# pananananas/MVD

Hardware: AMD Instinct MI355X
Metric: UNet forward-passes/sec @512x512 SD2.1+MV adapter (higher is better)
Workload: dtype bf16; 1 GPU; cfg4: configs[3]/[4]: 8 objects x 4 target views per GPU (32 pairs), camera FiLM + cross-view adapter; pairs_per_gpu=32, global_pairs=32, latent=64x64x4, image=512x512, forward=cold, hip_graph=False, q2_statistics=replica-local, parallelism=dp1 (pairs sharded by object), weights=synthetic seeded, SD2.1 shapes (865.9M UNet x2 + 99.2M adapter + 19.1M camera), encoder_weights=distinct

## Files before the change

### include/mvd_hip.h

```cpp
#ifndef MVD_HIP_H
#define MVD_HIP_H
#include <stddef.h>
#include <stdint.h>

#ifdef __cplusplus
extern "C" {
#endif

#define MVD_MAX_LEVELS 4

typedef struct {
  int in_channels;
  int out_channels;
  int num_levels;
  int block_out_channels[MVD_MAX_LEVELS];
  int num_heads[MVD_MAX_LEVELS];
  int layers_per_block;
  int cross_attention_dim;
  int norm_num_groups;
  float norm_eps;
  int cam_output_dim;
  int cam_hidden_dim;
  int simple_cam_encoder;
  float cam_modulation_strength;
} mvd_config_t;

typedef struct mvd_engine mvd_engine_t;

const char* mvd_last_error(void);

int mvd_engine_create(const mvd_config_t* cfg, mvd_engine_t** out);
int mvd_engine_destroy(mvd_engine_t* e);

int mvd_engine_set_weight(mvd_engine_t* e, int set, const char* slot, const void* ptr, int64_t numel, int dtype);
int mvd_engine_clear_weights(mvd_engine_t* e, int set);

int64_t mvd_engine_workspace_bytes(mvd_engine_t* e, int batch, int height, int width, int text_len, int ref_batch);
int64_t mvd_engine_refcache_bytes(mvd_engine_t* e, int ref_batch, int height, int width, int keep_features);
int mvd_engine_bind_workspace(mvd_engine_t* e, void* ws, int64_t ws_bytes, void* refcache, int64_t refcache_bytes);

enum {
  MVD_USE_CAMERA = 1,
  MVD_USE_IMAGE = 2,
  MVD_REUSE_REF = 4,
  MVD_KEEP_FEATURES = 8,
  MVD_SHARE_REF = 16
};


typedef struct {
  int batch;
  int height, width;
  int text_len;
  const float* sample;
  const float* timesteps;
  const float* text;
  const float* source_camera;
  const float* target_camera;
  int cam_rows;
  int cam_batch;
  const float* fourier_proj;
  const float* source_latents;
  const float* encoder_text;
  int ref_batch;
  int flags;
  float* out;
  int views;
} mvd_forward_args_t;

int mvd_unet_forward(mvd_engine_t* e, const mvd_forward_args_t* args, void* stream);
int64_t mvd_engine_workspace_bytes_args(mvd_engine_t* e, const mvd_forward_args_t* args);

int mvd_unet_forward_objects(mvd_engine_t* e, const mvd_forward_args_t* args, int objects, void* stream);
int64_t mvd_engine_workspace_bytes_objects(mvd_engine_t* e, const mvd_forward_args_t* args, int objects);

int mvd_unet_forward_ragged(mvd_engine_t* e, const mvd_forward_args_t* args, const int* view_counts, int objects, void* stream);
int64_t mvd_engine_workspace_bytes_ragged(mvd_engine_t* e, const mvd_forward_args_t* args, const int* view_counts, int objects);

int64_t mvd_engine_reference_pixels(mvd_engine_t* e, int height, int width);
int mvd_engine_reference_encode(mvd_engine_t* e, const mvd_forward_args_t* args, float* local_stats, void* stream);
int mvd_engine_reference_finish(mvd_engine_t* e, const float* mean_k, void* stream);

int mvd_engine_set_graph(mvd_engine_t* e, int enable);

int mvd_engine_share_encoder_weights(mvd_engine_t* e, int enable);

int mvd_engine_set_freeu(mvd_engine_t* e, float s1, float s2, float b1, float b2);
int mvd_engine_clear_freeu(mvd_engine_t* e);

int mvd_engine_set_profiling(mvd_engine_t* e, int enable);
int mvd_engine_profile_summary(mvd_engine_t* e, int cap, int* cls, int* launches, double* ms, double* flops, double* bytes);
int mvd_engine_profile_shapes(mvd_engine_t* e, char* buf_host, int cap);

int mvd_engine_num_features(mvd_engine_t* e);
int mvd_engine_feature_shape(mvd_engine_t* e, int idx, int* channels, int* height, int* width);
int mvd_engine_get_feature(mvd_engine_t* e, int idx, float* out_nchw, void* stream);
int mvd_engine_encode_cameras(mvd_engine_t* e, const float* source_camera, const float* target_camera, int cam_rows,
                              int batch, const float* fourier_proj, float* out_emb, void* stream);
int mvd_engine_apply_modulation(mvd_engine_t* e, const char* name, const float* emb, int batch, const float* x_nchw,
                                int channels, int hw, float* out_nchw, void* stream);
int mvd_engine_get_camera_embedding(mvd_engine_t* e, float* out, void* stream);
int mvd_engine_film_params(mvd_engine_t* e, const float* emb, int cam_batch, int out_rows, float* out, void* stream);
int mvd_engine_time_projection(mvd_engine_t* e, const float* timesteps, int batch, float* out, void* stream);

int mvd_op_linear(const void* a, const void* a2, int k1, int k2, const void* w, const float* bias, const float* rowvec,
                  int ld_rowvec, int rows_per_batch, const void* res, float alpha, int geglu, void* out, int out_f32,
                  int m, int n, int force_cfg, int splitk, float* splitk_ws ,
                  void* stream);
int mvd_op_ln_linear(const void* x, int k, const void* w_folded, const float* c1, const float* c2, float eps, int geglu,
                     void* out, int m, int n, void* stream);
int mvd_op_linear_xs(const void* x, int ldx, const void* w_packed, int m, int k, int units, int geglu, int ln, float ln_eps,
                     const void* res, int ldres, void* out, int ldo, int csplit, void* stream);
int mvd_op_conv3x3_ws(const void* x, int batch, int h, int w, int c, const void* w_packed, const float* bias, const float* rowvec,
                      int ld_rowvec, const void* res, const void* sc, const void* sc2, int sc_c1, int sc_c2, void* out, int n,
                      int variant, void* stream);
int mvd_op_conv3x3(const void* x, int batch, int in_h, int in_w, int cin, int stride, int upsample, int asym_pad, const void* w,
                   const float* bias, const float* rowvec, int ld_rowvec, const void* res, const void* sc, const void* sc2,
                   int sc_c1, int sc_c2, void* out, int cout, int force_cfg, int splitk, float* splitk_ws, void* stream);
int mvd_op_conv3x3_up4(const void* x, int batch, int in_h, int in_w, int cin, const void* w4, const float* bias, void* out, int cout,
                       int force_cfg, void* stream);
int mvd_op_attention(const void* q, const void* k, const void* v, void* o, int batch, int heads, int nq, int nk, int ldq,
                     int ldk, int ldv, int ldo, float scale, void* stream);
int mvd_op_attention_grouped(const void* q, const void* k, const void* v, void* o, int batch, int heads, int nq, int nk, int ldq,
                             int ldk, int ldv, int ldo, float scale, int kv_group, void* stream);
int mvd_op_attention_objects(const void* q, const void* k, const void* v, void* o, int batch, int heads, int nq, int nk, int ldq,
                             int ldk, int ldv, int ldo, float scale, int kv_group, int kv_objects, void* stream);
int mvd_op_attention_mapped(const void* q, const void* k, const void* v, void* o, int batch, int heads, int nq, int nk, int ldq,
                            int ldk, int ldv, int ldo, float scale, const int* kv_index_host, int kv_elements, void* stream);
int64_t mvd_op_attention_split_ws_bytes(int batch, int heads, int nq, int nsplit);
int mvd_op_attention_split(const void* q, const void* k, const void* v, void* o, int batch, int heads, int nq, int nk, int ldq,
                           int ldk, int ldv, int ldo, int nsplit, void* ws, void* stream);
int mvd_op_groupnorm(const void* x0, const void* x1, int c0, int c1, int batch, int hw, int groups, float eps,
                     const float* gamma, const float* beta, int silu, void* y, float* ws, void* stream);
int mvd_op_layernorm(const void* x, int rows, int c, float eps, const float* gamma, const float* beta, void* y,
                     void* stream);
int mvd_op_refnorm(const void* x, int batch, int hw, int c, void* y, void* stream);
int mvd_op_refnorm_grouped(const void* x, int batch, int group, int hw, int c, void* y, void* stream);
int mvd_op_film(const void* x, int batch, int hw, int c, const float* scale, const float* shift, void* y, void* stream);
int mvd_op_conv_in(const void* x, int batch, int h, int w, int cin, const float* wt, const float* bias, int cout, void* y,
                   void* stream);
int mvd_op_conv_out(const void* x, int batch, int h, int w, int c, const void* wt, const float* bias, int cout, float* y,
                    void* stream);
int mvd_op_nchw_to_nhwc(const float* x, int batch, int c, int hw, const float* scale, const float* shift, void* y,
                        void* stream);
int mvd_op_nhwc_to_nchw(const void* x, int batch, int hw, int c, float* y, void* stream);
int mvd_op_f32_to_bf16(const float* x, int64_t n, void* y, void* stream);
int mvd_op_skinny_linear(const float* x, int ldx, int batch, int k, const void* w, int wbf16, const float* bias, int n, int act_in,
                         float* y, int ldy, void* stream);
int mvd_op_timestep_embedding(const float* t, int batch, int dim, float* y, void* stream);
int mvd_op_camera_features(const float* src, const float* tgt, int batch, int cam_rows, int nfreq, float max_freq, float* rflat,
                           float* enc, void* stream);
int mvd_op_layernorm_f32(const float* x, int rows, int c, float eps, const float* gamma, const float* beta, int silu, int nseg,
                         float* y, void* stream);
int mvd_op_skinny_linear_grouped(const float* x, int ldx, int xseg, int batch, int k, const float* w, const float* bias, int n,
                                 const int* seg_end, int nseg, float* y, int ldy, void* stream);
int mvd_op_film_params(const float* raw, int batch, int dim, float strength, float* scale, float* shift, int out_rows,
                       void* stream);
int mvd_op_film_params_grouped(const float* raw, int batch, const int* seg_end, int nseg, float strength, float* out, int out_rows,
                               void* stream);
int mvd_op_im2col_in(const float* x, int batch, int c, int h, int w, const float* scale, const float* shift, int ld_ss, void* y,
                     void* stream);
int mvd_op_film_nchw_f32(const float* x, int batch, int c, int hw, const float* scale, const float* shift, float* y, void* stream);
int mvd_gemm_num_configs(void);
int mvd_debug_last_gemm_plan(int* out);
int mvd_debug_last_attention_plan(int* out);
int mvd_debug_last_groupnorm_plan(int* out);
long mvd_debug_up4_launches(void);
int mvd_debug_last_gemm_nowait(void);
int mvd_debug_pick_splitk(int m, int n, int k, int geglu);
int mvd_debug_pick_splitk_conv(int m, int n, int k);
int mvd_debug_dense_route(int m, int n, int k1, int k2, int* out);
int mvd_gemm_sm_num_tiles(void);
int mvd_debug_set_attention_nw(int nw_log2);
int mvd_debug_ragged_tables(const int* view_counts, int objects, int g, int* adapter, int* text);
int mvd_debug_attention_mapped_grouped(const void* q, const void* k, const void* v, void* o, int batch, int heads, int nq, int nk,
                                       int ldq, int ldk, int ldv, int ldo, float scale, int kv_group, int kv_objects,
                                       const int* kv_index_host, int kv_elements, void* stream);
typedef enum {
  MVD_DBG_NO_SM_LN_FOLD = 1,
  MVD_DBG_SM_NO_SPLITK = 2,
  MVD_DBG_NO_SM = 4,
  MVD_DBG_NO_SPLIT_KV = 8,
  MVD_DBG_ONE_STREAM = 16,
  MVD_DBG_SINGLE_STREAM_POLICY = 32,
  MVD_DBG_SIDE_DEFAULT_PRIORITY = 64,
  MVD_DBG_NO_XS = 128,
  MVD_DBG_NO_WS = 256,
  MVD_DBG_WS_SMALL_MAPS = 512,
  MVD_DBG_WS_BLOCK64 = 1024,
  MVD_DBG_WS_NO_SHORTCUT = 2048,
  MVD_DBG_WS_NOT_IN_ENCODER = 4096,
  MVD_DBG_WS_ONLY_IN_ENCODER = 8192,
  MVD_DBG_WS_THEN_TILED = 16384,
  MVD_DBG_WS_CHECK = 32768,
  MVD_DBG_GRAPH_ONE_STREAM = 65536,
  MVD_DBG_PP_ROW_MAJOR = 131072,
  MVD_DBG_NO_DEEP_CONV_SPLIT = 262144,
  MVD_DBG_LATE_FROM_UP1 = 524288,
  MVD_DBG_NO_UP4 = 1048576,
  MVD_DBG_GN_ONE_PASS = 2097152,
  MVD_DBG_FORK_LATE = 4194304,
  MVD_DBG_SKINNY_VECTOR = 8388608
} mvd_debug_flag_t;
int mvd_debug_set_flags(int flags);

int mvd_op_ddpm_step(const float* model_out, const float* sample, const float* noise, float c0, float c1, float c2,
                     float c3, float sigma, float* out, int64_t n, void* stream);
int mvd_op_cfg_combine(const float* uncond_cond, float guidance_scale, float* out, int64_t n_half, void* stream);
int mvd_op_sampler_step(const float* model_out, int guided, float guidance_scale, const float* sample, const float* x0_prev,
                        const float* noise, float a0, float a1, float p, float q, float r, float sigma, float* out,
                        float* x0_out, int64_t n, void* stream);
int mvd_op_cfg_rescale(const float* uncond_cond, float guidance_scale, float guidance_rescale, float* out, int64_t rows,
                       int64_t n_row, void* stream);
int mvd_op_sampler_step_rescaled(const float* model_out, float guidance_scale, float guidance_rescale, const float* sample,
                                 const float* x0_prev, const float* noise, float a0, float a1, float p, float q, float r,
                                 float sigma, float* out, float* x0_out, int64_t rows, int64_t n_row, void* stream);
int mvd_debug_cfg_rescale_plan(int64_t n_row, int* out);
int mvd_op_apg(const float* uncond_cond, float guidance_scale, float eta, float norm_threshold, float momentum,
               float guidance_rescale, float* momentum_buffer, float* out, int64_t rows, int64_t n_row, void* stream);
int mvd_op_sampler_step_apg(const float* model_out, float guidance_scale, float eta, float norm_threshold, float momentum,
                            float guidance_rescale, int space, float* momentum_buffer, const float* sample, const float* x0_prev,
                            const float* noise, float a0, float a1, float p, float q, float r, float sigma, float* out,
                            float* x0_out, int64_t rows, int64_t n_row, void* stream);
int mvd_debug_apg_plan(int64_t n_row, int* out);

int mvd_op_freeu(const void* hidden, int C, const void* skip, int Cs, int B, int H, int W, float b, float s, void* hidden_out,
                 void* skip_out, void* stream);

int mvd_op_add_noise(const float* x0, const float* noise, const int32_t* timesteps, const float* sqrt_ac, const float* sqrt_1mac,
                     int num_train_timesteps, float* noisy, float* velocity, int batch, int64_t per_sample, void* stream);
int64_t mvd_op_noise_loss_ws_bytes(int batch, int64_t per_sample);
int mvd_op_noise_loss(const float* pred, const float* noise, const float* x0, const float* noisy, const int32_t* timesteps,
                      const float* sqrt_ac, const float* sqrt_1mac, const float* snr, int num_train_timesteps, int prediction_type,
                      float snr_gamma, float* denoised, float* result, int batch, int64_t per_sample, void* ws, int64_t ws_bytes,
                      void* stream);
int64_t mvd_op_image_metrics_ws_bytes(int n, int c, int h, int w, int want_ssim);
int mvd_op_image_metrics(const float* x, const float* y, int n, int c, int h, int w, float data_range, int want_ssim, float* result,
                         float* per_image, void* ws, int64_t ws_bytes, void* stream);

typedef struct {
  int in_channels;
  int latent_channels;
  int num_levels;
  int block_out_channels[MVD_MAX_LEVELS];
  int layers_per_block;
  int norm_num_groups;
  float norm_eps;
} mvd_vae_config_t;
typedef struct mvd_vae mvd_vae_t;
int mvd_vae_create(const mvd_vae_config_t* cfg, mvd_vae_t** out);
int mvd_vae_destroy(mvd_vae_t* v);
int mvd_vae_set_weight(mvd_vae_t* v, const char* slot, const void* ptr, int64_t numel, int dtype);
int64_t mvd_vae_workspace_bytes(mvd_vae_t* v, int batch, int height, int width, int decode);
int mvd_vae_bind_workspace(mvd_vae_t* v, void* ws, int64_t ws_bytes);
int mvd_vae_encode(mvd_vae_t* v, const float* image_nchw, int batch, int height, int width, float* moments, void* stream);
int mvd_vae_decode(mvd_vae_t* v, const float* latents_nchw, int batch, int height, int width, float* image, void* stream);
int64_t mvd_vae_mid_attention_workspace_bytes(mvd_vae_t* v, int decoder, int batch, int height, int width);
int mvd_vae_mid_attention(mvd_vae_t* v, int decoder, const void* x_nhwc_bf16, int batch, int height, int width, void* out_nhwc_bf16,
                          void* stream);
int mvd_op_softmax_rows(const float* s, int rows, int n, void* p_bf16, void* stream);
int mvd_op_gaussian_sample(const float* moments, const float* noise, int batch, int channels, int hw, float scale, float* out,
                           void* stream);

typedef struct {
  int vocab_size;
  int hidden_size;
  int intermediate_size;
  int num_layers;
  int num_heads;
  int max_positions;
  float layer_norm_eps;
  int act;
} mvd_text_config_t;
typedef struct mvd_text mvd_text_t;
int mvd_text_create(const mvd_text_config_t* cfg, mvd_text_t** out);
int mvd_text_destroy(mvd_text_t* t);
int mvd_text_set_weight(mvd_text_t* t, const char* slot, const void* ptr, int64_t numel, int dtype);
int64_t mvd_text_workspace_bytes(mvd_text_t* t, int batch, int seq_len);
int mvd_text_bind_workspace(mvd_text_t* t, void* ws, int64_t bytes);
int mvd_text_encode(mvd_text_t* t, const int32_t* ids, int batch, int seq_len, float* out, void* stream);
int mvd_op_attention_causal(const void* q, const void* k, const void* v, void* o, int batch, int heads, int n, int ldq, int ldk,
                            int ldv, int ldo, float scale, void* stream);

typedef struct {
  int image_size;
  int patch_size;
  int hidden_size;
  int intermediate_size;
  int num_layers;
  int num_heads;
  int projection_dim;
  float layer_norm_eps;
  int act;
} mvd_vision_config_t;
typedef struct mvd_vision mvd_vision_t;
int mvd_vision_create(const mvd_vision_config_t* cfg, mvd_vision_t** out);
int mvd_vision_destroy(mvd_vision_t* v);
int mvd_vision_set_weight(mvd_vision_t* v, const char* slot, const void* ptr, int64_t numel, int dtype);
int64_t mvd_vision_workspace_bytes(mvd_vision_t* v, int batch, int h, int w, int resize_to);
int mvd_vision_bind_workspace(mvd_vision_t* v, void* ws, int64_t bytes);
int mvd_vision_preprocess(mvd_vision_t* v, const float* images_nchw, int batch, int h, int w, int quantize, int resize_to, int crop,
                          const float* mean, const float* std_, int want_patches, float* pixel_values, void* stream);
int64_t mvd_vision_patch_rows_offset(mvd_vision_t* v);
int mvd_vision_encode(mvd_vision_t* v, const float* pixel_values, int batch, float* last_hidden_out, float* embeds_out,
                      float* embeds_norm_out, void* stream);
int mvd_op_clip_pool_project(const float* hidden, const float* delta, const int32_t* ids, int batch, int tokens, int hidden_size,
                             int eos_token_id, const float* ln_gamma, const float* ln_beta, float eps, const float* proj_w, int proj_dim,
                             float* embeds, float* embeds_norm, void* stream);
int mvd_op_clip_cosine(const float* a, const float* b, int batch, int dim, float* per_row_out, float* mean_out, void* stream);

typedef struct mvd_vgg mvd_vgg_t;
int mvd_vgg_create(mvd_vgg_t** out);
int mvd_vgg_destroy(mvd_vgg_t* v);
int mvd_vgg_set_weight(mvd_vgg_t* v, const char* slot, const void* ptr, int64_t numel, int dtype);
int64_t mvd_vgg_workspace_bytes(mvd_vgg_t* v, int images, int h, int w);
int mvd_vgg_bind_workspace(mvd_vgg_t* v, void* ws, int64_t bytes);
int mvd_vgg_features(mvd_vgg_t* v, const float* images_nchw, int images, int h, int w, float* feat_out_nhwc, void* const* taps, void* stream);
int mvd_vgg_perceptual(mvd_vgg_t* v, const float* x, const float* y, int pairs, int h, int w, float* loss_out, float* per_pair_out, void* stream);
int mvd_op_conv3x3_relu(const void* x, int batch, int in_h, int in_w, int cin, const void* w, const float* bias, void* out, int cout, int relu,
// ... 65 lines not shown
```

### mvd_amd/_lib.py

```python
from __future__ import annotations

import ctypes as C
import enum
import os

HERE = os.path.dirname(os.path.abspath(__file__))
LIB_PATH = os.environ.get("MVD_HIP_LIB") or os.path.join(HERE, "libmvd_hip.so")

MVD_MAX_LEVELS = 4
MVD_USE_CAMERA, MVD_USE_IMAGE, MVD_REUSE_REF, MVD_KEEP_FEATURES, MVD_SHARE_REF = 1, 2, 4, 8, 16


class MvdError(RuntimeError):
    pass


class DebugFlag(enum.IntFlag):
    NO_SM_LN_FOLD = 1
    SM_NO_SPLITK = 2
    NO_SM = 4
    NO_SPLIT_KV = 8
    ONE_STREAM = 16
    SINGLE_STREAM_POLICY = 32
    SIDE_DEFAULT_PRIORITY = 64
    NO_XS = 128
    NO_WS = 256
    WS_SMALL_MAPS = 512
    WS_BLOCK64 = 1024
    WS_NO_SHORTCUT = 2048
    WS_NOT_IN_ENCODER = 4096
    WS_ONLY_IN_ENCODER = 8192
    WS_THEN_TILED = 16384
    WS_CHECK = 32768
    GRAPH_ONE_STREAM = 65536
    PP_ROW_MAJOR = 131072
    NO_DEEP_CONV_SPLIT = 262144
    LATE_FROM_UP1 = 524288
    NO_UP4 = 1048576
    GN_ONE_PASS = 2097152
    FORK_LATE = 4194304
    SKINNY_VECTOR = 8388608


class mvd_config_t(C.Structure):
    _fields_ = [
        ("in_channels", C.c_int), ("out_channels", C.c_int), ("num_levels", C.c_int),
        ("block_out_channels", C.c_int * MVD_MAX_LEVELS), ("num_heads", C.c_int * MVD_MAX_LEVELS),
        ("layers_per_block", C.c_int), ("cross_attention_dim", C.c_int), ("norm_num_groups", C.c_int),
        ("norm_eps", C.c_float), ("cam_output_dim", C.c_int), ("cam_hidden_dim", C.c_int),
        ("simple_cam_encoder", C.c_int), ("cam_modulation_strength", C.c_float),
    ]


class mvd_vae_config_t(C.Structure):
    _fields_ = [
        ("in_channels", C.c_int), ("latent_channels", C.c_int), ("num_levels", C.c_int),
        ("block_out_channels", C.c_int * MVD_MAX_LEVELS), ("layers_per_block", C.c_int), ("norm_num_groups", C.c_int),
        ("norm_eps", C.c_float),
    ]


class mvd_text_config_t(C.Structure):
    _fields_ = [
        ("vocab_size", C.c_int), ("hidden_size", C.c_int), ("intermediate_size", C.c_int), ("num_layers", C.c_int),
        ("num_heads", C.c_int), ("max_positions", C.c_int), ("layer_norm_eps", C.c_float), ("act", C.c_int),
    ]


class mvd_vision_config_t(C.Structure):
    _fields_ = [
        ("image_size", C.c_int), ("patch_size", C.c_int), ("hidden_size", C.c_int), ("intermediate_size", C.c_int),
        ("num_layers", C.c_int), ("num_heads", C.c_int), ("projection_dim", C.c_int), ("layer_norm_eps", C.c_float), ("act", C.c_int),
    ]


class mvd_forward_args_t(C.Structure):
    _fields_ = [
        ("batch", C.c_int), ("height", C.c_int), ("width", C.c_int), ("text_len", C.c_int),
        ("sample", C.c_void_p), ("timesteps", C.c_void_p), ("text", C.c_void_p),
        ("source_camera", C.c_void_p), ("target_camera", C.c_void_p), ("cam_rows", C.c_int), ("cam_batch", C.c_int),
        ("fourier_proj", C.c_void_p), ("source_latents", C.c_void_p), ("encoder_text", C.c_void_p),
        ("ref_batch", C.c_int), ("flags", C.c_int), ("out", C.c_void_p), ("views", C.c_int),
    ]


_SIGS = {
    "mvd_last_error": (C.c_char_p, []),
    "mvd_engine_create": (C.c_int, [C.POINTER(mvd_config_t), C.POINTER(C.c_void_p)]),
    "mvd_engine_destroy": (C.c_int, [C.c_void_p]),
    "mvd_engine_set_weight": (C.c_int, [C.c_void_p, C.c_int, C.c_char_p, C.c_void_p, C.c_int64, C.c_int]),
    "mvd_engine_clear_weights": (C.c_int, [C.c_void_p, C.c_int]),
    "mvd_engine_workspace_bytes": (C.c_int64, [C.c_void_p, C.c_int, C.c_int, C.c_int, C.c_int, C.c_int]),
    "mvd_engine_workspace_bytes_args": (C.c_int64, [C.c_void_p, C.POINTER(mvd_forward_args_t)]),
    "mvd_engine_workspace_bytes_objects": (C.c_int64, [C.c_void_p, C.POINTER(mvd_forward_args_t), C.c_int]),
    "mvd_engine_refcache_bytes": (C.c_int64, [C.c_void_p, C.c_int, C.c_int, C.c_int, C.c_int]),
    "mvd_engine_bind_workspace": (C.c_int, [C.c_void_p, C.c_void_p, C.c_int64, C.c_void_p, C.c_int64]),
    "mvd_unet_forward": (C.c_int, [C.c_void_p, C.POINTER(mvd_forward_args_t), C.c_void_p]),
    "mvd_unet_forward_objects": (C.c_int, [C.c_void_p, C.POINTER(mvd_forward_args_t), C.c_int, C.c_void_p]),
    "mvd_unet_forward_ragged": (C.c_int, [C.c_void_p, C.POINTER(mvd_forward_args_t), C.POINTER(C.c_int), C.c_int, C.c_void_p]),
    "mvd_engine_workspace_bytes_ragged": (C.c_int64, [C.c_void_p, C.POINTER(mvd_forward_args_t), C.POINTER(C.c_int), C.c_int]),
    "mvd_debug_ragged_tables": (C.c_int, [C.POINTER(C.c_int), C.c_int, C.c_int, C.POINTER(C.c_int), C.POINTER(C.c_int)]),
    "mvd_engine_set_profiling": (C.c_int, [C.c_void_p, C.c_int]),
    "mvd_engine_profile_summary": (C.c_int, [C.c_void_p, C.c_int, C.POINTER(C.c_int), C.POINTER(C.c_int),
                                             C.POINTER(C.c_double), C.POINTER(C.c_double), C.POINTER(C.c_double)]),
    "mvd_engine_profile_shapes": (C.c_int, [C.c_void_p, C.c_char_p, C.c_int]),
    "mvd_engine_set_graph": (C.c_int, [C.c_void_p, C.c_int]),
    "mvd_engine_reference_pixels": (C.c_int64, [C.c_void_p, C.c_int, C.c_int]),
    "mvd_engine_reference_encode": (C.c_int, [C.c_void_p, C.POINTER(mvd_forward_args_t), C.c_void_p, C.c_void_p]),
    "mvd_engine_reference_finish": (C.c_int, [C.c_void_p, C.c_void_p, C.c_void_p]),
    "mvd_engine_share_encoder_weights": (C.c_int, [C.c_void_p, C.c_int]),
    "mvd_engine_num_features": (C.c_int, [C.c_void_p]),
    "mvd_engine_feature_shape": (C.c_int, [C.c_void_p, C.c_int, C.POINTER(C.c_int), C.POINTER(C.c_int), C.POINTER(C.c_int)]),
    "mvd_engine_get_feature": (C.c_int, [C.c_void_p, C.c_int, C.c_void_p, C.c_void_p]),
    "mvd_engine_encode_cameras": (C.c_int, [C.c_void_p, C.c_void_p, C.c_void_p, C.c_int, C.c_int, C.c_void_p, C.c_void_p, C.c_void_p]),
    "mvd_engine_apply_modulation": (C.c_int, [C.c_void_p, C.c_char_p, C.c_void_p, C.c_int, C.c_void_p, C.c_int, C.c_int, C.c_void_p, C.c_void_p]),
    "mvd_engine_get_camera_embedding": (C.c_int, [C.c_void_p, C.c_void_p, C.c_void_p]),
    "mvd_engine_film_params": (C.c_int, [C.c_void_p, C.c_void_p, C.c_int, C.c_int, C.c_void_p, C.c_void_p]),
    "mvd_engine_time_projection": (C.c_int, [C.c_void_p, C.c_void_p, C.c_int, C.c_void_p, C.c_void_p]),
    "mvd_op_linear": (C.c_int, [C.c_void_p, C.c_void_p, C.c_int, C.c_int, C.c_void_p, C.c_void_p, C.c_void_p, C.c_int,
                                C.c_int, C.c_void_p, C.c_float, C.c_int, C.c_void_p, C.c_int, C.c_int, C.c_int, C.c_int,
                                C.c_int, C.c_void_p, C.c_void_p]),
    "mvd_op_ln_linear": (C.c_int, [C.c_void_p, C.c_int, C.c_void_p, C.c_void_p, C.c_void_p, C.c_float, C.c_int, C.c_void_p,
                                   C.c_int, C.c_int, C.c_void_p]),
    "mvd_op_linear_xs": (C.c_int, [C.c_void_p, C.c_int, C.c_void_p, C.c_int, C.c_int, C.c_int, C.c_int, C.c_int, C.c_float,
                                   C.c_void_p, C.c_int, C.c_void_p, C.c_int, C.c_int, C.c_void_p]),
    "mvd_op_conv3x3_ws": (C.c_int, [C.c_void_p, C.c_int, C.c_int, C.c_int, C.c_int, C.c_void_p, C.c_void_p, C.c_void_p, C.c_int,
                                    C.c_void_p, C.c_void_p, C.c_void_p, C.c_int, C.c_int, C.c_void_p, C.c_int, C.c_int, C.c_void_p]),
    "mvd_op_conv3x3": (C.c_int, [C.c_void_p, C.c_int, C.c_int, C.c_int, C.c_int, C.c_int, C.c_int, C.c_int, C.c_void_p, C.c_void_p,
                                 C.c_void_p, C.c_int, C.c_void_p, C.c_void_p, C.c_void_p, C.c_int, C.c_int, C.c_void_p,
                                 C.c_int, C.c_int, C.c_int, C.c_void_p, C.c_void_p]),
    "mvd_op_attention": (C.c_int, [C.c_void_p, C.c_void_p, C.c_void_p, C.c_void_p, C.c_int, C.c_int, C.c_int, C.c_int,
                                   C.c_int, C.c_int, C.c_int, C.c_int, C.c_float, C.c_void_p]),
    "mvd_op_attention_grouped": (C.c_int, [C.c_void_p, C.c_void_p, C.c_void_p, C.c_void_p, C.c_int, C.c_int, C.c_int, C.c_int,
                                           C.c_int, C.c_int, C.c_int, C.c_int, C.c_float, C.c_int, C.c_void_p]),
    "mvd_op_attention_objects": (C.c_int, [C.c_void_p, C.c_void_p, C.c_void_p, C.c_void_p, C.c_int, C.c_int, C.c_int, C.c_int,
                                           C.c_int, C.c_int, C.c_int, C.c_int, C.c_float, C.c_int, C.c_int, C.c_void_p]),
    "mvd_op_attention_mapped": (C.c_int, [C.c_void_p, C.c_void_p, C.c_void_p, C.c_void_p, C.c_int, C.c_int, C.c_int, C.c_int,
                                          C.c_int, C.c_int, C.c_int, C.c_int, C.c_float, C.POINTER(C.c_int), C.c_int, C.c_void_p]),
    "mvd_debug_attention_mapped_grouped": (C.c_int, [C.c_void_p, C.c_void_p, C.c_void_p, C.c_void_p, C.c_int, C.c_int, C.c_int, C.c_int,
                                                     C.c_int, C.c_int, C.c_int, C.c_int, C.c_float, C.c_int, C.c_int, C.POINTER(C.c_int),
                                                     C.c_int, C.c_void_p]),
    "mvd_op_attention_split_ws_bytes": (C.c_int64, [C.c_int, C.c_int, C.c_int, C.c_int]),
    "mvd_op_attention_split": (C.c_int, [C.c_void_p, C.c_void_p, C.c_void_p, C.c_void_p, C.c_int, C.c_int, C.c_int, C.c_int, C.c_int,
                                         C.c_int, C.c_int, C.c_int, C.c_int, C.c_void_p, C.c_void_p]),
    "mvd_op_groupnorm": (C.c_int, [C.c_void_p, C.c_void_p, C.c_int, C.c_int, C.c_int, C.c_int, C.c_int, C.c_float,
                                   C.c_void_p, C.c_void_p, C.c_int, C.c_void_p, C.c_void_p, C.c_void_p]),
    "mvd_op_layernorm": (C.c_int, [C.c_void_p, C.c_int, C.c_int, C.c_float, C.c_void_p, C.c_void_p, C.c_void_p, C.c_void_p]),
    "mvd_op_refnorm": (C.c_int, [C.c_void_p, C.c_int, C.c_int, C.c_int, C.c_void_p, C.c_void_p]),
    "mvd_op_refnorm_grouped": (C.c_int, [C.c_void_p, C.c_int, C.c_int, C.c_int, C.c_int, C.c_void_p, C.c_void_p]),
    "mvd_op_film": (C.c_int, [C.c_void_p, C.c_int, C.c_int, C.c_int, C.c_void_p, C.c_void_p, C.c_void_p, C.c_void_p]),
    "mvd_op_conv_in": (C.c_int, [C.c_void_p, C.c_int, C.c_int, C.c_int, C.c_int, C.c_void_p, C.c_void_p, C.c_int, C.c_void_p, C.c_void_p]),
    "mvd_op_conv_out": (C.c_int, [C.c_void_p, C.c_int, C.c_int, C.c_int, C.c_int, C.c_void_p, C.c_void_p, C.c_int, C.c_void_p, C.c_void_p]),
    "mvd_op_nchw_to_nhwc": (C.c_int, [C.c_void_p, C.c_int, C.c_int, C.c_int, C.c_void_p, C.c_void_p, C.c_void_p, C.c_void_p]),
    "mvd_op_nhwc_to_nchw": (C.c_int, [C.c_void_p, C.c_int, C.c_int, C.c_int, C.c_void_p, C.c_void_p]),
    "mvd_op_f32_to_bf16": (C.c_int, [C.c_void_p, C.c_int64, C.c_void_p, C.c_void_p]),
    "mvd_op_skinny_linear": (C.c_int, [C.c_void_p, C.c_int, C.c_int, C.c_int, C.c_void_p, C.c_int, C.c_void_p, C.c_int, C.c_int,
                                        C.c_void_p, C.c_int, C.c_void_p]),
    "mvd_op_timestep_embedding": (C.c_int, [C.c_void_p, C.c_int, C.c_int, C.c_void_p, C.c_void_p]),
    "mvd_op_camera_features": (C.c_int, [C.c_void_p, C.c_void_p, C.c_int, C.c_int, C.c_int, C.c_float, C.c_void_p, C.c_void_p, C.c_void_p]),
    "mvd_op_layernorm_f32": (C.c_int, [C.c_void_p, C.c_int, C.c_int, C.c_float, C.c_void_p, C.c_void_p, C.c_int, C.c_int, C.c_void_p,
                                       C.c_void_p]),
    "mvd_op_skinny_linear_grouped": (C.c_int, [C.c_void_p, C.c_int, C.c_int, C.c_int, C.c_int, C.c_void_p, C.c_void_p, C.c_int,
                                               C.POINTER(C.c_int), C.c_int, C.c_void_p, C.c_int, C.c_void_p]),
    "mvd_op_film_params": (C.c_int, [C.c_void_p, C.c_int, C.c_int, C.c_float, C.c_void_p, C.c_void_p, C.c_int, C.c_void_p]),
    "mvd_op_film_params_grouped": (C.c_int, [C.c_void_p, C.c_int, C.POINTER(C.c_int), C.c_int, C.c_float, C.c_void_p, C.c_int, C.c_void_p]),
    "mvd_op_im2col_in": (C.c_int, [C.c_void_p, C.c_int, C.c_int, C.c_int, C.c_int, C.c_void_p, C.c_void_p, C.c_int, C.c_void_p, C.c_void_p]),
    "mvd_op_film_nchw_f32": (C.c_int, [C.c_void_p, C.c_int, C.c_int, C.c_int, C.c_void_p, C.c_void_p, C.c_void_p, C.c_void_p]),
    "mvd_gemm_num_configs": (C.c_int, []),
    "mvd_debug_last_gemm_plan": (C.c_int, [C.POINTER(C.c_int)]),
    "mvd_debug_up4_launches": (C.c_long, []),
    "mvd_op_conv3x3_up4": (C.c_int, [C.c_void_p, C.c_int, C.c_int, C.c_int, C.c_int, C.c_void_p, C.c_void_p, C.c_void_p, C.c_int, C.c_int,
                                     C.c_void_p]),
    "mvd_debug_last_gemm_nowait": (C.c_int, []),
    "mvd_debug_last_attention_plan": (C.c_int, [C.POINTER(C.c_int)]),
    "mvd_debug_last_groupnorm_plan": (C.c_int, [C.POINTER(C.c_int)]),
    "mvd_debug_pick_splitk": (C.c_int, [C.c_int, C.c_int, C.c_int, C.c_int]),
    "mvd_debug_pick_splitk_conv": (C.c_int, [C.c_int, C.c_int, C.c_int]),
    "mvd_debug_dense_route": (C.c_int, [C.c_int, C.c_int, C.c_int, C.c_int, C.POINTER(C.c_int)]),
    "mvd_gemm_sm_num_tiles": (C.c_int, []),
    "mvd_debug_set_attention_nw": (C.c_int, [C.c_int]),
    "mvd_debug_set_flags": (C.c_int, [C.c_int]),
    "mvd_op_ddpm_step": (C.c_int, [C.c_void_p, C.c_void_p, C.c_void_p, C.c_float, C.c_float, C.c_float, C.c_float,
                                   C.c_float, C.c_void_p, C.c_int64, C.c_void_p]),
    "mvd_op_cfg_combine": (C.c_int, [C.c_void_p, C.c_float, C.c_void_p, C.c_int64, C.c_void_p]),
    "mvd_op_sampler_step": (C.c_int, [C.c_void_p, C.c_int, C.c_float, C.c_void_p, C.c_void_p, C.c_void_p, C.c_float, C.c_float,
                                      C.c_float, C.c_float, C.c_float, C.c_float, C.c_void_p, C.c_void_p, C.c_int64, C.c_void_p]),
    "mvd_op_cfg_rescale": (C.c_int, [C.c_void_p, C.c_float, C.c_float, C.c_void_p, C.c_int64, C.c_int64, C.c_void_p]),
    "mvd_op_sampler_step_rescaled": (C.c_int, [C.c_void_p, C.c_float, C.c_float, C.c_void_p, C.c_void_p, C.c_void_p, C.c_float,
                                               C.c_float, C.c_float, C.c_float, C.c_float, C.c_float, C.c_void_p, C.c_void_p,
                                               C.c_int64, C.c_int64, C.c_void_p]),
    "mvd_debug_cfg_rescale_plan": (C.c_int, [C.c_int64, C.POINTER(C.c_int)]),
    "mvd_op_apg": (C.c_int, [C.c_void_p, C.c_float, C.c_float, C.c_float, C.c_float, C.c_float, C.c_void_p, C.c_void_p, C.c_int64,
                             C.c_int64, C.c_void_p]),
    "mvd_op_sampler_step_apg": (C.c_int, [C.c_void_p, C.c_float, C.c_float, C.c_float, C.c_float, C.c_float, C.c_int, C.c_void_p,
                                          C.c_void_p, C.c_void_p, C.c_void_p, C.c_float, C.c_float, C.c_float, C.c_float, C.c_float,
                                          C.c_float, C.c_void_p, C.c_void_p, C.c_int64, C.c_int64, C.c_void_p]),
    "mvd_debug_apg_plan": (C.c_int, [C.c_int64, C.POINTER(C.c_int)]),
    "mvd_engine_set_freeu": (C.c_int, [C.c_void_p, C.c_float, C.c_float, C.c_float, C.c_float]),
    "mvd_engine_clear_freeu": (C.c_int, [C.c_void_p]),
    "mvd_op_freeu": (C.c_int, [C.c_void_p, C.c_int, C.c_void_p, C.c_int, C.c_int, C.c_int, C.c_int, C.c_float, C.c_float, C.c_void_p,
                               C.c_void_p, C.c_void_p]),
    "mvd_op_add_noise": (C.c_int, [C.c_void_p, C.c_void_p, C.c_void_p, C.c_void_p, C.c_void_p, C.c_int, C.c_void_p, C.c_void_p, C.c_int,
                                   C.c_int64, C.c_void_p]),
    "mvd_op_noise_loss_ws_bytes": (C.c_int64, [C.c_int, C.c_int64]),
    "mvd_op_noise_loss": (C.c_int, [C.c_void_p, C.c_void_p, C.c_void_p, C.c_void_p, C.c_void_p, C.c_void_p, C.c_void_p, C.c_void_p,
                                    C.c_int, C.c_int, C.c_float, C.c_void_p, C.c_void_p, C.c_int, C.c_int64, C.c_void_p, C.c_int64,
                                    C.c_void_p]),
    "mvd_op_image_metrics_ws_bytes": (C.c_int64, [C.c_int, C.c_int, C.c_int, C.c_int, C.c_int]),
    "mvd_op_image_metrics": (C.c_int, [C.c_void_p, C.c_void_p, C.c_int, C.c_int, C.c_int, C.c_int, C.c_float, C.c_int, C.c_void_p,
                                       C.c_void_p, C.c_void_p, C.c_int64, C.c_void_p]),
    "mvd_vae_create": (C.c_int, [C.POINTER(mvd_vae_config_t), C.POINTER(C.c_void_p)]),
    "mvd_vae_destroy": (C.c_int, [C.c_void_p]),
    "mvd_vae_set_weight": (C.c_int, [C.c_void_p, C.c_char_p, C.c_void_p, C.c_int64, C.c_int]),
    "mvd_vae_workspace_bytes": (C.c_int64, [C.c_void_p, C.c_int, C.c_int, C.c_int, C.c_int]),
    "mvd_vae_bind_workspace": (C.c_int, [C.c_void_p, C.c_void_p, C.c_int64]),
    "mvd_vae_encode": (C.c_int, [C.c_void_p, C.c_void_p, C.c_int, C.c_int, C.c_int, C.c_void_p, C.c_void_p]),
    "mvd_vae_decode": (C.c_int, [C.c_void_p, C.c_void_p, C.c_int, C.c_int, C.c_int, C.c_void_p, C.c_void_p]),
    "mvd_vae_mid_attention_workspace_bytes": (C.c_int64, [C.c_void_p, C.c_int, C.c_int, C.c_int, C.c_int]),
    "mvd_vae_mid_attention": (C.c_int, [C.c_void_p, C.c_int, C.c_void_p, C.c_int, C.c_int, C.c_int, C.c_void_p, C.c_void_p]),
    "mvd_op_softmax_rows": (C.c_int, [C.c_void_p, C.c_int, C.c_int, C.c_void_p, C.c_void_p]),
    "mvd_op_gaussian_sample": (C.c_int, [C.c_void_p, C.c_void_p, C.c_int, C.c_int, C.c_int, C.c_float, C.c_void_p, C.c_void_p]),
    "mvd_text_create": (C.c_int, [C.POINTER(mvd_text_config_t), C.POINTER(C.c_void_p)]),
    "mvd_text_destroy": (C.c_int, [C.c_void_p]),
    "mvd_text_set_weight": (C.c_int, [C.c_void_p, C.c_char_p, C.c_void_p, C.c_int64, C.c_int]),
    "mvd_text_workspace_bytes": (C.c_int64, [C.c_void_p, C.c_int, C.c_int]),
    "mvd_text_bind_workspace": (C.c_int, [C.c_void_p, C.c_void_p, C.c_int64]),
    "mvd_text_encode": (C.c_int, [C.c_void_p, C.c_void_p, C.c_int, C.c_int, C.c_void_p, C.c_void_p]),
    "mvd_op_attention_causal": (C.c_int, [C.c_void_p, C.c_void_p, C.c_void_p, C.c_void_p, C.c_int, C.c_int, C.c_int, C.c_int,
                                          C.c_int, C.c_int, C.c_int, C.c_float, C.c_void_p]),
    "mvd_vision_create": (C.c_int, [C.POINTER(mvd_vision_config_t), C.POINTER(C.c_void_p)]),
    "mvd_vision_destroy": (C.c_int, [C.c_void_p]),
    "mvd_vision_set_weight": (C.c_int, [C.c_void_p, C.c_char_p, C.c_void_p, C.c_int64, C.c_int]),
    "mvd_vision_workspace_bytes": (C.c_int64, [C.c_void_p, C.c_int, C.c_int, C.c_int, C.c_int]),
    "mvd_vision_bind_workspace": (C.c_int, [C.c_void_p, C.c_void_p, C.c_int64]),
    "mvd_vision_preprocess": (C.c_int, [C.c_void_p, C.c_void_p, C.c_int, C.c_int, C.c_int, C.c_int, C.c_int, C.c_int,
                                        C.POINTER(C.c_float), C.POINTER(C.c_float), C.c_int, C.c_void_p, C.c_void_p]),
    "mvd_vision_patch_rows_offset": (C.c_int64, [C.c_void_p]),
    "mvd_vision_encode": (C.c_int, [C.c_void_p, C.c_void_p, C.c_int, C.c_void_p, C.c_void_p, C.c_void_p, C.c_void_p]),
    "mvd_op_clip_pool_project": (C.c_int, [C.c_void_p, C.c_void_p, C.c_void_p, C.c_int, C.c_int, C.c_int, C.c_int, C.c_void_p,
                                           C.c_void_p, C.c_float, C.c_void_p, C.c_int, C.c_void_p, C.c_void_p, C.c_void_p]),
    "mvd_op_clip_cosine": (C.c_int, [C.c_void_p, C.c_void_p, C.c_int, C.c_int, C.c_void_p, C.c_void_p, C.c_void_p]),
    "mvd_vgg_create": (C.c_int, [C.POINTER(C.c_void_p)]),
    "mvd_vgg_destroy": (C.c_int, [C.c_void_p]),
    "mvd_vgg_set_weight": (C.c_int, [C.c_void_p, C.c_char_p, C.c_void_p, C.c_int64, C.c_int]),
    "mvd_vgg_workspace_bytes": (C.c_int64, [C.c_void_p, C.c_int, C.c_int, C.c_int]),
    "mvd_vgg_bind_workspace": (C.c_int, [C.c_void_p, C.c_void_p, C.c_int64]),
    "mvd_vgg_features": (C.c_int, [C.c_void_p, C.c_void_p, C.c_int, C.c_int, C.c_int, C.c_void_p, C.POINTER(C.c_void_p), C.c_void_p]),
    "mvd_vgg_perceptual": (C.c_int, [C.c_void_p, C.c_void_p, C.c_void_p, C.c_int, C.c_int, C.c_int, C.c_void_p, C.c_void_p, C.c_void_p]),
    "mvd_op_conv3x3_relu": (C.c_int, [C.c_void_p, C.c_int, C.c_int, C.c_int, C.c_int, C.c_void_p, C.c_void_p, C.c_void_p, C.c_int, C.c_int,
                                      C.c_int, C.c_int, C.c_int, C.c_void_p, C.c_void_p]),
    "mvd_op_linear_relu": (C.c_int, [C.c_void_p, C.c_int, C.c_void_p, C.c_void_p, C.c_void_p, C.c_int, C.c_int, C.c_int, C.c_int, C.c_int,
                                     C.c_int, C.c_void_p, C.c_void_p]),
    "mvd_op_maxpool2x2": (C.c_int, [C.c_void_p, C.c_int, C.c_int, C.c_int, C.c_int, C.c_void_p, C.c_void_p]),
    "mvd_op_sqdiff_mean_ws_bytes": (C.c_int64, [C.c_int, C.c_int64]),
    "mvd_op_sqdiff_mean": (C.c_int, [C.c_void_p, C.c_void_p, C.c_int, C.c_int64, C.c_void_p, C.c_void_p, C.c_void_p, C.c_int64, C.c_void_p]),
    "mvd_lpips_create": (C.c_int, [C.POINTER(C.c_void_p)]),
    "mvd_lpips_destroy": (C.c_int, [C.c_void_p]),
    "mvd_lpips_set_weight": (C.c_int, [C.c_void_p, C.c_char_p, C.c_void_p, C.c_int64, C.c_int]),
    "mvd_lpips_workspace_bytes": (C.c_int64, [C.c_void_p, C.c_int, C.c_int, C.c_int]),
    "mvd_lpips_bind_workspace": (C.c_int, [C.c_void_p, C.c_void_p, C.c_int64]),
    "mvd_lpips_features": (C.c_int, [C.c_void_p, C.c_void_p, C.c_int, C.c_int, C.c_int, C.POINTER(C.c_void_p), C.c_void_p]),
    "mvd_lpips_distance": (C.c_int, [C.c_void_p, C.c_void_p, C.c_void_p, C.c_int, C.c_int, C.c_int, C.c_int, C.c_void_p, C.c_void_p,
                                     C.c_void_p, C.c_void_p]),
    "mvd_op_im2col_patch": (C.c_int, [C.c_void_p, C.c_int, C.c_int, C.c_int, C.c_int, C.POINTER(C.c_float), C.POINTER(C.c_float), C.c_void_p,
                                      C.c_void_p]),
    "mvd_op_maxpool3x3s2": (C.c_int, [C.c_void_p, C.c_int, C.c_int, C.c_int, C.c_int, C.c_void_p, C.c_void_p]),
    "mvd_op_lpips_head_ws_bytes": (C.c_int64, [C.c_int, C.POINTER(C.c_int), C.c_int]),
    "mvd_op_lpips_head": (C.c_int, [C.c_int, C.POINTER(C.c_void_p), C.POINTER(C.c_void_p), C.POINTER(C.c_int), C.POINTER(C.c_int),
                                    C.POINTER(C.c_int), C.POINTER(C.c_int), C.POINTER(C.c_void_p), C.c_int, C.c_void_p, C.c_void_p, C.c_void_p,
                                    C.c_void_p, C.c_int64, C.c_void_p]),
    "mvd_fid_create": (C.c_int, [C.POINTER(C.c_int), C.c_int, C.POINTER(C.c_int), C.c_int, C.POINTER(C.c_char_p), C.c_int, C.c_int, C.c_int,
                                 C.POINTER(C.c_void_p)]),
    "mvd_fid_destroy": (C.c_int, [C.c_void_p]),
    "mvd_fid_set_weight": (C.c_int, [C.c_void_p, C.c_char_p, C.c_void_p, C.c_int64, C.c_int]),
    "mvd_fid_feature_dim": (C.c_int, [C.c_void_p]),
    "mvd_fid_workspace_bytes": (C.c_int64, [C.c_void_p, C.c_int]),
    "mvd_fid_bind_workspace": (C.c_int, [C.c_void_p, C.c_void_p, C.c_int64]),
    "mvd_fid_features": (C.c_int, [C.c_void_p, C.c_void_p, C.c_int, C.c_int, C.c_int, C.c_int, C.c_void_p, C.c_void_p]),
    "mvd_fid_update": (C.c_int, [C.c_void_p, C.c_void_p, C.c_int, C.c_int, C.c_int, C.c_int, C.c_void_p, C.c_void_p, C.c_void_p]),
    "mvd_op_conv_relu_slice": (C.c_int, [C.c_void_p, C.c_int, C.c_int, C.c_int, C.c_int, C.c_int, C.c_int, C.c_void_p, C.c_void_p, C.c_int, C.c_int,
                                         C.c_int, C.c_int, C.c_int, C.c_int, C.c_void_p, C.c_int, C.c_int, C.c_int, C.c_void_p]),
    "mvd_op_pool3x3_slice": (C.c_int, [C.c_void_p, C.c_int, C.c_int, C.c_int, C.c_int, C.c_int, C.c_int, C.c_int, C.c_void_p, C.c_int, C.c_int,
                                       C.c_void_p]),
    "mvd_op_resize_tf1": (C.c_int, [C.c_void_p, C.c_int, C.c_int, C.c_int, C.c_int, C.c_void_p, C.c_void_p]),
    "mvd_op_global_mean": (C.c_int, [C.c_void_p, C.c_int, C.c_int, C.c_int, C.c_void_p, C.c_void_p]),
    "mvd_op_feature_stats": (C.c_int, [C.c_void_p, C.c_int, C.c_int, C.c_void_p, C.c_void_p, C.c_void_p]),
    "mvd_op_kid_workspace_bytes": (C.c_int64, [C.c_int, C.c_int]),
    "mvd_op_kid_mmd": (C.c_int, [C.c_void_p, C.c_int, C.c_void_p, C.c_int, C.c_int, C.c_void_p, C.c_int, C.c_int, C.c_int, C.c_double, C.c_double,
                                 C.c_void_p, C.c_int64, C.c_void_p, C.c_void_p, C.c_void_p]),
    "mvd_op_fc_logits": (C.c_int, [C.c_void_p, C.c_int, C.c_int, C.c_void_p, C.c_int, C.c_void_p, C.c_void_p]),
    "mvd_op_inception_score_workspace_bytes": (C.c_int64, [C.c_int, C.c_int, C.c_int]),
    "mvd_op_inception_score": (C.c_int, [C.c_void_p, C.c_int, C.c_int, C.c_void_p, C.c_int, C.c_void_p, C.c_int64, C.c_void_p, C.POINTER(C.c_int),
                                         C.c_void_p]),
    "mvd_op_knn_radii_workspace_bytes": (C.c_int64, [C.c_int, C.c_int, C.c_int]),
    "mvd_op_knn_radii": (C.c_int, [C.c_void_p, C.c_int, C.c_int, C.c_int, C.c_int, C.c_void_p, C.c_void_p, C.c_void_p, C.c_int64, C.c_void_p]),
    "mvd_op_manifold_counts": (C.c_int, [C.c_void_p, C.c_int, C.c_void_p, C.c_int, C.c_int, C.c_void_p, C.c_int, C.c_void_p, C.c_void_p, C.c_void_p]),
    "mvd_op_image_frontend_spans": (C.c_int, [C.POINTER(C.c_int)]),
    "mvd_op_image_frontend_workspace_bytes": (C.c_int64, [C.c_int, C.c_int, C.c_int, C.c_int, C.c_int, C.c_int]),
    "mvd_op_image_frontend": (C.c_int, [C.c_void_p, C.c_int, C.c_int, C.c_int, C.c_int, C.c_int, C.c_int, C.c_void_p, C.c_void_p, C.c_void_p,
                                        C.c_int64, C.c_void_p]),
}

EXPORTED_SYMBOLS = tuple(_SIGS)

_lib = None


def lib() -> C.CDLL:
    global _lib
    if _lib is None:
        if not os.path.exists(LIB_PATH):
            raise MvdError(
                f"{LIB_PATH} not found: build the HIP extension first "
                "(python -c 'import __graft_entry__ as g; g.build()' or python mvd_amd/_build.py)")
        import torch
        l = C.CDLL(LIB_PATH)
        for name, (res, args) in _SIGS.items():
            fn = getattr(l, name)
            fn.restype = res
            fn.argtypes = args
        _lib = l
    return _lib


def last_error() -> str:
    return lib().mvd_last_error().decode()


# ... 58 lines not shown
```

### mvd_amd/csrc/engine.hip

```cpp
#include <math.h>
#include <stdio.h>
#include <stdlib.h>
#include <string.h>

#include <mutex>
#include <string>
#include <unordered_map>
#include <vector>

#include "host_util.h"
#include "ragged.h"

int mvd_launch_silu_to_bf16(const float* x, int64_t n, bf16_t* y, hipStream_t s);

static int g_debug_flags = 0;
extern "C" int mvd_debug_set_flags(int flags) { g_debug_flags = flags; return 0; }
int mvd_debug_flags() { return g_debug_flags; }

namespace {

struct FeatureInfo { std::string name; int level; int C; int heads; std::string key;  };
constexpr int MVD_REF_ONLY_INTERNAL = 1 << 30;

}
// ... 1545 lines not shown
  if (splitk > 1 && force_cfg >= 100) return op_sm_splitk(g, s, force_cfg);
  return launch_tiled(g, s, force_cfg);
}
int mvd_op_linear(const void* a, const void* a2, int k1, int k2, const void* w, const float* bias, const float* rowvec,
                  int ld_rowvec, int rows_per_batch, const void* res, float alpha, int geglu, void* out, int out_f32, int m,
                  int n, int force_cfg, int splitk, float* splitk_ws, void* stream) {
  const int on = geglu ? n / 2 : n;
  MvdGemmArgs g = gemm_dense((const bf16_t*)a, (const bf16_t*)a2, k1, k2, m, (const bf16_t*)w, 0, bias, n, out, on);
  if (rows_per_batch > 0) g.rows_per_batch = g.outW = rows_per_batch;
  g.rowvec = rowvec; g.ld_rowvec = ld_rowvec; g.res = (const bf16_t*)res; g.ldres = on; g.alpha = alpha; g.geglu = geglu; g.out_f32 = out_f32;
  return op_launch(g, force_cfg, splitk, splitk_ws, (hipStream_t)stream);
}

int mvd_op_ln_linear(const void* x, int k, const void* w_folded, const float* c1, const float* c2, float eps, int geglu,
                     void* out, int m, int n, void* stream) {
  MvdGemmArgs g = gemm_dense((const bf16_t*)x, nullptr, k, 0, m, (const bf16_t*)w_folded, 0, c2, n, out, geglu ? n / 2 : n);
  g.ln_c1 = c1; g.ln_eps = eps; g.geglu = geglu; g.ldres = g.ldo;
  if (!c1 || !c2) { mvd_set_error("mvd_op_ln_linear: c1 and c2 are required"); return -1; }
  if (!mvd_gemm_ln_fold_ok(g)) {
    int tile = 0, ns = 0, S = 1;
    if (mvd_gemm_sm_plan(g, &tile, &ns, &S) && S == 1) {
      g_mvd_last_gemm.cfg = 100 + 10 * tile + ns; g_mvd_last_gemm.splitk = 1;
      return mvd_launch_gemm_sm(g, (hipStream_t)stream, tile, ns);
    }
    mvd_set_error("mvd_op_ln_linear: M=%d N=%d K=%d geglu=%d is not a shape of the fused LayerNorm GEMMs", m, n, k, geglu);
    return -1;
  }
  return mvd_launch_gemm(g, (hipStream_t)stream);
}

int mvd_op_conv3x3(const void* x, int batch, int in_h, int in_w, int cin, int stride, int upsample, int asym_pad, const void* w,
                   const float* bias, const float* rowvec, int ld_rowvec, const void* res, const void* sc, const void* sc2,
                   int sc_c1, int sc_c2, void* out, int cout, int force_cfg, int splitk, float* splitk_ws, void* stream) {
  const int oh = upsample ? in_h * 2 : (stride == 2 ? (in_h + 1) / 2 : in_h);
  const int ow = upsample ? in_w * 2 : (stride == 2 ? (in_w + 1) / 2 : in_w);
  MvdGemmArgs g = gemm_conv3((const bf16_t*)x, in_h, in_w, cin, stride, upsample, asym_pad, (const bf16_t*)sc, (const bf16_t*)sc2, sc_c1, sc_c2,
                             (const bf16_t*)w, bias, batch, oh, ow, cout, out);
  g.rowvec = rowvec; g.ld_rowvec = ld_rowvec; g.res = (const bf16_t*)res;
  return op_launch(g, force_cfg, splitk, splitk_ws, (hipStream_t)stream);
}

int mvd_op_conv3x3_up4(const void* x, int batch, int in_h, int in_w, int cin, const void* w4, const float* bias, void* out, int cout,
                       int force_cfg, void* stream) {
  if (!x || !w4 || !out || batch <= 0 || in_h <= 0 || in_w <= 0 || cin <= 0 || cout <= 0) { mvd_set_error("mvd_op_conv3x3_up4: bad argument"); return -1; }
  MvdGemmArgs g = gemm_conv3((const bf16_t*)x, in_h, in_w, cin, 1, 1, 0, nullptr, nullptr, 0, 0, (const bf16_t*)w4, bias, batch, 2 * in_h, 2 * in_w,
                             cout, out);
  gemm_conv3_to_up4(g);
  g.splitk = 1;
  return mvd_launch_gemm(g, (hipStream_t)stream, force_cfg);
}

int mvd_op_attention(const void* q, const void* k, const void* v, void* o, int batch, int heads, int nq, int nk, int ldq,
                     int ldk, int ldv, int ldo, float scale, void* stream) {
  MvdAttnArgs a; memset(&a, 0, sizeof(a));
  a.nprob = 1; a.batch = batch; a.heads = heads; a.scale = scale;
  a.prescaled = scale == 0.f;
  a.p[0] = {(const bf16_t*)q, (const bf16_t*)k, (const bf16_t*)v, (bf16_t*)o, ldq, ldk, ldv, ldo,
            (int64_t)nq * ldq, (int64_t)nk * ldk, (int64_t)nk * ldv, (int64_t)nq * ldo, nq, nk};
  return mvd_launch_attention(a, (hipStream_t)stream);
}

int mvd_op_attention_grouped(const void* q, const void* k, const void* v, void* o, int batch, int heads, int nq, int nk, int ldq,
                             int ldk, int ldv, int ldo, float scale, int kv_group, void* stream) {
  return mvd_op_attention_objects(q, k, v, o, batch, heads, nq, nk, ldq, ldk, ldv, ldo, scale, kv_group, 0, stream);
}

int mvd_op_attention_objects(const void* q, const void* k, const void* v, void* o, int batch, int heads, int nq, int nk, int ldq,
                             int ldk, int ldv, int ldo, float scale, int kv_group, int kv_objects, void* stream) {
  MvdAttnArgs a; memset(&a, 0, sizeof(a));
  a.nprob = 1; a.batch = batch; a.heads = heads; a.scale = scale;
  a.prescaled = scale == 0.f;
  a.p[0] = {(const bf16_t*)q, (const bf16_t*)k, (const bf16_t*)v, (bf16_t*)o, ldq, ldk, ldv, ldo,
            (int64_t)nq * ldq, (int64_t)nk * ldk, (int64_t)nk * ldv, (int64_t)nq * ldo, nq, nk};
  a.kv_group[0] = kv_group; a.kv_objects[0] = kv_objects;
  return mvd_launch_attention(a, (hipStream_t)stream);
}

int64_t mvd_op_attention_split_ws_bytes(int batch, int heads, int nq, int nsplit) {
  MvdAttnArgs a; memset(&a, 0, sizeof(a));
  a.nprob = 1; a.batch = batch; a.heads = heads; a.p[0].nq = nq;
  return (int64_t)mvd_attention_split_ws_bytes(a, nsplit) + (int64_t)mvd_attention_split_counters(a) * 4 + 256;
}
static int* g_op_kvi = nullptr; static size_t g_op_kvi_cap = 0; static std::mutex g_op_kvi_mu;
static int attention_mapped(const void* q, const void* k, const void* v, void* o, int batch, int heads, int nq, int nk, int ldq, int ldk,
                            int ldv, int ldo, float scale, int kv_group, int kv_objects, const int* kv_index_host, int kv_elements,
                            void* stream) {
  if (batch <= 0) { mvd_set_error("attention: bad problem count/batch/heads"); return -1; }
  if (mvd_attention_check_index(kv_index_host, batch, kv_elements)) return -1;
  if (kv_group > 1 || kv_objects > 1) { mvd_set_error("attention: problem 0 sets a K/V table together with K/V group %d / objects %d", kv_group, kv_objects); return -1; }
  MvdAttnArgs a; memset(&a, 0, sizeof(a));
  a.nprob = 1; a.batch = batch; a.heads = heads; a.scale = scale;
  a.prescaled = scale == 0.f;
  a.p[0] = {(const bf16_t*)q, (const bf16_t*)k, (const bf16_t*)v, (bf16_t*)o, ldq, ldk, ldv, ldo,
            (int64_t)nq * ldq, (int64_t)nk * ldk, (int64_t)nk * ldv, (int64_t)nq * ldo, nq, nk};
  std::lock_guard<std::mutex> lk(g_op_kvi_mu);
  if ((size_t)batch > g_op_kvi_cap) {
    if (g_op_kvi) (void)hipFree(g_op_kvi);
    g_op_kvi = nullptr; g_op_kvi_cap = 0;
    const size_t cap = (size_t)batch < 256 ? 256 : (size_t)batch;
    if (hipMalloc((void**)&g_op_kvi, cap * sizeof(int)) != hipSuccess) { mvd_set_error("attention: hipMalloc of the K/V table failed"); return -3; }
    g_op_kvi_cap = cap;
  }
  if (hipMemcpyAsync(g_op_kvi, kv_index_host, (size_t)batch * sizeof(int), hipMemcpyHostToDevice, (hipStream_t)stream) != hipSuccess) { mvd_set_error("attention: upload of the K/V table failed"); return -3; }
  a.kv_index[0] = g_op_kvi; a.kv_group[0] = kv_group; a.kv_objects[0] = kv_objects;
  return mvd_launch_attention(a, (hipStream_t)stream);
}
int mvd_op_attention_mapped(const void* q, const void* k, const void* v, void* o, int batch, int heads, int nq, int nk, int ldq,
                            int ldk, int ldv, int ldo, float scale, const int* kv_index_host, int kv_elements, void* stream) {
  return attention_mapped(q, k, v, o, batch, heads, nq, nk, ldq, ldk, ldv, ldo, scale, 0, 0, kv_index_host, kv_elements, stream);
}
extern "C" int mvd_debug_attention_mapped_grouped(const void* q, const void* k, const void* v, void* o, int batch, int heads, int nq, int nk,
                                                  int ldq, int ldk, int ldv, int ldo, float scale, int kv_group, int kv_objects,
                                                  const int* kv_index_host, int kv_elements, void* stream) {
  return attention_mapped(q, k, v, o, batch, heads, nq, nk, ldq, ldk, ldv, ldo, scale, kv_group, kv_objects, kv_index_host, kv_elements, stream);
}

extern "C" int mvd_debug_ragged_tables(const int* view_counts, int objects, int g, int* adapter, int* text) {
  if (!view_counts || !adapter || !text || objects < 1 || g < 1 || g > 2) { mvd_set_error("ragged_tables: bad argument"); return -1; }
  const int R = mvd_ragged_rows(view_counts, objects);
  if (R < 0) { mvd_set_error("ragged_tables: every object needs at least one view"); return -1; }
  mvd_ragged_build_tables(view_counts, objects, g, adapter, text);
  if (mvd_attention_check_index(adapter, g * R, g * objects) || mvd_attention_check_index(text, g * R, g * objects)) return -1;
  return g * R;
}

int mvd_op_attention_split(const void* q, const void* k, const void* v, void* o, int batch, int heads, int nq, int nk, int ldq,
                           int ldk, int ldv, int ldo, int nsplit, void* ws, void* stream) {
  MvdAttnArgs a; memset(&a, 0, sizeof(a));
  a.nprob = 1; a.batch = batch; a.heads = heads; a.scale = 0.f; a.prescaled = 1;
  a.p[0] = {(const bf16_t*)q, (const bf16_t*)k, (const bf16_t*)v, (bf16_t*)o, ldq, ldk, ldv, ldo,
            (int64_t)nq * ldq, (int64_t)nk * ldk, (int64_t)nk * ldv, (int64_t)nq * ldo, nq, nk};
  if (nsplit > 1) {
    if (!ws) { mvd_set_error("op_attention_split: null workspace"); return -1; }
    const size_t pb = (mvd_attention_split_ws_bytes(a, nsplit) + 255) & ~size_t(255);
    a.nsplit = nsplit; a.split_ws = ws; a.split_cnt = reinterpret_cast<unsigned int*>(reinterpret_cast<char*>(ws) + pb);
    if (hipMemsetAsync(a.split_cnt, 0, (size_t)mvd_attention_split_counters(a) * 4, (hipStream_t)stream) != hipSuccess) { mvd_set_error("op_attention_split: hipMemsetAsync failed"); return -3; }
  }
  return mvd_launch_attention(a, (hipStream_t)stream);
}

int mvd_op_groupnorm(const void* x0, const void* x1, int c0, int c1, int batch, int hw, int groups, float eps,
                     const float* gamma, const float* beta, int silu, void* y, float* ws, void* stream) {
  return mvd_launch_groupnorm((const bf16_t*)x0, (const bf16_t*)x1, c0, c1, batch, hw, groups, eps, gamma, beta, silu, (bf16_t*)y, ws, (hipStream_t)stream);
}
int mvd_op_layernorm(const void* x, int rows, int c, float eps, const float* gamma, const float* beta, void* y, void* stream) {
  return mvd_launch_layernorm((const bf16_t*)x, rows, c, eps, gamma, beta, (bf16_t*)y, (hipStream_t)stream);
}
int mvd_op_refnorm(const void* x, int batch, int hw, int c, void* y, void* stream) {
  return mvd_launch_refnorm((const bf16_t*)x, batch, hw, c, (bf16_t*)y, (hipStream_t)stream);
}
int mvd_op_refnorm_grouped(const void* x, int batch, int group, int hw, int c, void* y, void* stream) {
  return mvd_launch_refnorm_grouped((const bf16_t*)x, batch, group, hw, c, (bf16_t*)y, (hipStream_t)stream);
}
int mvd_op_film(const void* x, int batch, int hw, int c, const float* scale, const float* shift, void* y, void* stream) {
  return mvd_launch_film((const bf16_t*)x, batch, hw, c, scale, shift, c, (bf16_t*)y, (hipStream_t)stream);
}
int mvd_op_conv_in(const void* x, int batch, int h, int w, int cin, const float* wt, const float* bias, int cout, void* y, void* stream) {
  return mvd_launch_conv_in((const bf16_t*)x, batch, h, w, cin, wt, bias, cout, (bf16_t*)y, (hipStream_t)stream);
}
int mvd_op_conv_out(const void* x, int batch, int h, int w, int c, const void* wt, const float* bias, int cout, float* y, void* stream) {
  return mvd_launch_conv_out((const bf16_t*)x, batch, h, w, c, (const bf16_t*)wt, bias, cout, y, (hipStream_t)stream);
}
int mvd_op_nchw_to_nhwc(const float* x, int batch, int c, int hw, const float* scale, const float* shift, void* y, void* stream) {
  return mvd_launch_nchw_to_nhwc(x, batch, c, hw, scale, shift, c, (bf16_t*)y, (hipStream_t)stream);
}
int mvd_op_nhwc_to_nchw(const void* x, int batch, int hw, int c, float* y, void* stream) {
  return mvd_launch_nhwc_to_nchw_f32((const bf16_t*)x, batch, hw, c, y, (hipStream_t)stream);
}
int mvd_op_f32_to_bf16(const float* x, int64_t n, void* y, void* stream) {
  return mvd_launch_f32_to_bf16(x, n, (bf16_t*)y, (hipStream_t)stream);
}
int mvd_op_skinny_linear(const float* x, int ldx, int batch, int k, const void* w, int wbf16, const float* bias, int n, int act_in,
                         float* y, int ldy, void* stream) {
  return mvd_launch_skinny_linear(x, ldx, batch, k, w, wbf16, bias, n, act_in, y, ldy, (hipStream_t)stream);
}
int mvd_op_timestep_embedding(const float* t, int batch, int dim, float* y, void* stream) {
  return mvd_launch_timestep_embedding(t, batch, dim, y, (hipStream_t)stream);
}
int mvd_op_camera_features(const float* src, const float* tgt, int batch, int cam_rows, int nfreq, float max_freq, float* rflat, float* enc,
                           void* stream) {
  return mvd_launch_camera_features(src, tgt, batch, cam_rows, nfreq, max_freq, rflat, enc, (hipStream_t)stream);
}
int mvd_op_layernorm_f32(const float* x, int rows, int c, float eps, const float* gamma, const float* beta, int silu, int nseg, float* y,
                         void* stream) {
  return mvd_launch_layernorm_f32(x, rows, c, eps, gamma, beta, silu, y, (hipStream_t)stream, nseg);
}
static int op_seg_table(const int* seg_end, int nseg, MvdSegTable* seg, const char* what) {
  if (!seg_end || nseg < 1 || nseg > 16) { mvd_set_error("%s: 1..16 segment ends", what); return -1; }
  memset(seg, 0, sizeof(*seg));
  seg->n = nseg;
  for (int g = 0; g < nseg; ++g) {
    if (seg_end[g] <= (g ? seg_end[g - 1] : 0)) { mvd_set_error("%s: segment ends must increase", what); return -1; }
    seg->end[g] = seg_end[g];
  }
  return 0;
}
int mvd_op_skinny_linear_grouped(const float* x, int ldx, int xseg, int batch, int k, const float* w, const float* bias, int n,
                                 const int* seg_end, int nseg, float* y, int ldy, void* stream) {
  MvdSegTable seg;
  if (int r = op_seg_table(seg_end, nseg, &seg, "skinny_linear_grouped")) return r;
  return mvd_launch_skinny_linear_grouped(x, ldx, xseg, batch, k, w, bias, n, seg, y, ldy, (hipStream_t)stream);
}
int mvd_op_film_params(const float* raw, int batch, int dim, float strength, float* scale, float* shift, int out_rows, void* stream) {
  return mvd_launch_film_params(raw, batch, dim, strength, scale, shift, out_rows, (hipStream_t)stream);
}
int mvd_op_film_params_grouped(const float* raw, int batch, const int* seg_end, int nseg, float strength, float* out, int out_rows,
                               void* stream) {
  MvdSegTable seg;
  if (int r = op_seg_table(seg_end, nseg, &seg, "film_params_grouped")) return r;
  return mvd_launch_film_params_grouped(raw, batch, seg, strength, out, out_rows, (hipStream_t)stream);
}
int mvd_op_im2col_in(const float* x, int batch, int c, int h, int w, const float* scale, const float* shift, int ld_ss, void* y,
                     void* stream) {
  return mvd_launch_im2col_in(x, batch, c, h, w, scale, shift, ld_ss, (bf16_t*)y, (hipStream_t)stream);
}
int mvd_op_film_nchw_f32(const float* x, int batch, int c, int hw, const float* scale, const float* shift, float* y, void* stream) {
  return mvd_launch_film_nchw_f32(x, batch, c, hw, scale, shift, y, (hipStream_t)stream);
}

}
```

### mvd_amd/csrc/misc.hip

```cpp
#include <stdarg.h>
#include <stdio.h>
#include <stdlib.h>
#include "host_util.h"

static thread_local char g_err[512] = "";
void mvd_set_error(const char* fmt, ...) {
  va_list ap;
  va_start(ap, fmt);
  vsnprintf(g_err, sizeof(g_err), fmt, ap);
  va_end(ap);
}
extern "C" const char* mvd_last_error(void) { return g_err; }

namespace {

__global__ void nchw_to_nhwc_kernel(const float* __restrict__ x, int c, int hw, const float* __restrict__ scale,
                                    const float* __restrict__ shift, int ld_ss, bf16_t* __restrict__ y, long total) {
  const long i = (long)blockIdx.x * blockDim.x + threadIdx.x;
  if (i >= total) return;
  const int ch = i % c;
  const long bp = i / c;
  const int p = bp % hw;
  const int b = bp / hw;
  float v = x[((size_t)b * c + ch) * hw + p];
  if (scale) v = v * scale[(size_t)b * ld_ss + ch] + shift[(size_t)b * ld_ss + ch];
  y[i] = f2bf(v);
}

__global__ void nhwc_to_nchw_f32_kernel(const bf16_t* __restrict__ x, int hw, int c, float* __restrict__ y, long total) {
  const long i = (long)blockIdx.x * blockDim.x + threadIdx.x;
  if (i >= total) return;
  const int p = i % hw;
  const long bc = i / hw;
  const int ch = bc % c;
  const int b = bc / c;
  y[i] = bf2f(x[((size_t)b * hw + p) * c + ch]);
}

__global__ void film_kernel(const bf16_t* __restrict__ x, int hw, int c, const float* __restrict__ scale,
                            const float* __restrict__ shift, int ld_ss, bf16_t* __restrict__ y, long nvec) {
  const int vec = c >> 3;
  for (long e = (long)blockIdx.x * blockDim.x + threadIdx.x; e < nvec; e += (long)gridDim.x * blockDim.x) {
    const int v = e % vec;
    const long bp = e / vec;
    const int b = bp / hw;
    const u32x4 in = *reinterpret_cast<const u32x4*>(x + e * 8);
    const float* sc = scale + (size_t)b * ld_ss + v * 8;
    const float* sf = shift + (size_t)b * ld_ss + v * 8;
    u32x4 o;
#pragma unroll
    for (int j = 0; j < 4; ++j)
      o[j] = pack2bf(fmaf(bflo(in[j]), sc[2 * j], sf[2 * j]), fmaf(bfhi(in[j]), sc[2 * j + 1], sf[2 * j + 1]));
    *reinterpret_cast<u32x4*>(y + e * 8) = o;
  }
}

__global__ void conv_in_kernel(const bf16_t* __restrict__ x, int h, int w, int cin, const float* __restrict__ wt,
                               const float* __restrict__ bias, int cout, bf16_t* __restrict__ y, long total) {
  const long i = (long)blockIdx.x * blockDim.x + threadIdx.x;
  if (i >= total) return;
  const int ng = cout >> 3;
  const int g = i % ng;
  const long bp = i / ng;
  const int hw = h * w;
  const int p = bp % hw;
  const int b = bp / hw;
  const int oy = p / w, ox = p % w;
  float acc[8];
#pragma unroll
  for (int j = 0; j < 8; ++j) acc[j] = bias[g * 8 + j];
  for (int tap = 0; tap < 9; ++tap) {
    const int iy = oy + tap / 3 - 1, ix = ox + tap % 3 - 1;
    if ((unsigned)iy >= (unsigned)h || (unsigned)ix >= (unsigned)w) continue;
    const bf16_t* xp = x + ((size_t)b * hw + iy * w + ix) * cin;
    for (int ci = 0; ci < cin; ++ci) {
      const float xv = bf2f(xp[ci]);
#pragma unroll
      for (int j = 0; j < 8; ++j) acc[j] = fmaf(xv, wt[((size_t)(g * 8 + j) * 9 + tap) * cin + ci], acc[j]);
    }
  }
  u32x4 o = {pack2bf(acc[0], acc[1]), pack2bf(acc[2], acc[3]), pack2bf(acc[4], acc[5]), pack2bf(acc[6], acc[7])};
  *reinterpret_cast<u32x4*>(y + bp * cout + g * 8) = o;
}

__global__ __launch_bounds__(256) void conv_out_kernel(const bf16_t* __restrict__ x, int batch, int h, int w, int c,
                                                        const bf16_t* __restrict__ wt, const float* __restrict__ bias,
                                                        int cout, float* __restrict__ y) {
  const int lane = threadIdx.x & 63;
  const long pix = (long)blockIdx.x * 4 + (threadIdx.x >> 6);
  const int hw = h * w;
  if (pix >= (long)batch * hw) return;
  const int b = pix / hw, p = pix % hw;
  const int oy = p / w, ox = p % w;
  const int vec = c >> 3;
  float acc[8];
#pragma unroll
  for (int j = 0; j < 8; ++j) acc[j] = 0.f;
  for (int q = lane; q < 9 * vec; q += 64) {
    const int tap = q / vec, v = q % vec;
    const int iy = oy + tap / 3 - 1, ix = ox + tap % 3 - 1;
    if ((unsigned)iy >= (unsigned)h || (unsigned)ix >= (unsigned)w) continue;
    const u32x4 xv = *reinterpret_cast<const u32x4*>(x + ((size_t)b * hw + iy * w + ix) * c + v * 8);
#pragma unroll
    for (int co = 0; co < 8; ++co) {
      if (co < cout) {
        const u32x4 wv = *reinterpret_cast<const u32x4*>(wt + ((size_t)co * 9 + tap) * c + v * 8);
        float a = acc[co];
#pragma unroll
        for (int j = 0; j < 4; ++j) {
          a = fmaf(bflo(xv[j]), bflo(wv[j]), a);
          a = fmaf(bfhi(xv[j]), bfhi(wv[j]), a);
        }
        acc[co] = a;
      }
    }
  }
#pragma unroll
  for (int co = 0; co < 8; ++co) {
    if (co < cout) {
      const float t = wave_sum(acc[co]);
      if (lane == 0) y[((size_t)b * cout + co) * hw + p] = t + bias[co];
    }
  }
}

__global__ void f32_to_bf16_kernel(const float* __restrict__ x, long n, bf16_t* __restrict__ y) {
  for (long i = (long)blockIdx.x * blockDim.x + threadIdx.x; i < n; i += (long)gridDim.x * blockDim.x) y[i] = f2bf(x[i]);
}

template <bool WBF16>
__global__ __launch_bounds__(256) void skinny_linear_kernel(const float* __restrict__ x, int ldx, int batch, int k,
                                                             const void* __restrict__ wv, const float* __restrict__ bias,
                                                             int n, int act_in, float* __restrict__ y, int ldy) {
  constexpr int BC = 32;
  const int lane = threadIdx.x & 63;
  const int o = blockIdx.x * 4 + (threadIdx.x >> 6);
  if (o >= n) return;
  const bool vec = !WBF16 && (k & 3) == 0 && (ldx & 3) == 0;
  for (int b0 = 0; b0 < batch; b0 += BC) {
    float acc[BC];
#pragma unroll
    for (int j = 0; j < BC; ++j) acc[j] = 0.f;
    if (vec) {
      const float* wr = reinterpret_cast<const float*>(wv) + (size_t)o * k;
      for (int kk = lane * 4; kk < k; kk += 256) {
        const f32x4 w4 = *reinterpret_cast<const f32x4*>(wr + kk);
#pragma unroll
        for (int j = 0; j < BC; ++j) {
          if (b0 + j < batch) {
            f32x4 x4 = *reinterpret_cast<const f32x4*>(x + (size_t)(b0 + j) * ldx + kk);
            if (act_in == 1) { x4[0] = silu_f(x4[0]); x4[1] = silu_f(x4[1]); x4[2] = silu_f(x4[2]); x4[3] = silu_f(x4[3]); }
            acc[j] = fmaf(x4[0], w4[0], fmaf(x4[1], w4[1], fmaf(x4[2], w4[2], fmaf(x4[3], w4[3], acc[j]))));
          }
        }
      }
    } else {
      for (int kk = lane; kk < k; kk += 64) {
        float wgt;
        if (WBF16) wgt = bf2f(reinterpret_cast<const bf16_t*>(wv)[(size_t)o * k + kk]);
        else wgt = reinterpret_cast<const float*>(wv)[(size_t)o * k + kk];
#pragma unroll
        for (int j = 0; j < BC; ++j) {
          if (b0 + j < batch) {
            float xv = x[(size_t)(b0 + j) * ldx + kk];
            if (act_in == 1) xv = silu_f(xv);
            acc[j] = fmaf(xv, wgt, acc[j]);
          }
        }
      }
    }
#pragma unroll
    for (int j = 0; j < BC; ++j) {
      if (b0 + j < batch) {
        const float t = wave_sum(acc[j]);
        if (lane == 0) y[(size_t)(b0 + j) * ldy + o] = t + (bias ? bias[o] : 0.f);
      }
    }
  }
}

template <bool WBF16, int F, bool GROUPED = false>
__global__ __launch_bounds__(256) void skinny_linear_vec_kernel(const float* __restrict__ x, int ldx, int batch, int k,
                                                                 const void* __restrict__ wv, const float* __restrict__ bias,
                                                                 int n, int act_in, float* __restrict__ y, int ldy,
                                                                 const MvdSegTable seg = MvdSegTable{}, int xseg = 0) {
  constexpr int BC = 32;
  constexpr int KV = WBF16 ? 8 : 4;
  const int lane = threadIdx.x & 63;
  const int o0 = (blockIdx.x * 4 + (threadIdx.x >> 6)) * F;
  if (o0 >= n) return;
  if constexpr (GROUPED) {
    int g = 0;
    while (g + 1 < seg.n && o0 >= seg.end[g]) ++g;
    x += (size_t)g * xseg;
  }
  for (int b0 = 0; b0 < batch; b0 += BC) {
    float acc[BC][F];
#pragma unroll
    for (int j = 0; j < BC; ++j)
#pragma unroll
      for (int f = 0; f < F; ++f) acc[j][f] = 0.f;
    for (int kk = lane * KV; kk < k; kk += 64 * KV) {
      float w[F][KV];
#pragma unroll
      for (int f = 0; f < F; ++f) {
        const int o = o0 + f < n ? o0 + f : n - 1;
        if (WBF16) {
          const u32x4 r = *reinterpret_cast<const u32x4*>(reinterpret_cast<const bf16_t*>(wv) + (size_t)o * k + kk);
#pragma unroll
          for (int e = 0; e < 4; ++e) { w[f][2 * e] = bflo(r[e]); w[f][2 * e + 1] = bfhi(r[e]); }
        } else {
          const f32x4 r = *reinterpret_cast<const f32x4*>(reinterpret_cast<const float*>(wv) + (size_t)o * k + kk);
#pragma unroll
          for (int e = 0; e < 4; ++e) w[f][e] = r[e];
        }
      }
#pragma unroll
      for (int j = 0; j < BC; ++j) {
        const int jr = b0 + j < batch ? b0 + j : batch - 1;
        float xv[KV];
#pragma unroll
        for (int q = 0; q < KV / 4; ++q) {
          const f32x4 x4 = *reinterpret_cast<const f32x4*>(x + (size_t)jr * ldx + kk + 4 * q);
#pragma unroll
          for (int e = 0; e < 4; ++e) xv[4 * q + e] = act_in == 1 ? silu_f(x4[e]) : x4[e];
        }
#pragma unroll
        for (int f = 0; f < F; ++f)
#pragma unroll
          for (int e = 0; e < KV; ++e) acc[j][f] = fmaf(xv[e], w[f][e], acc[j][f]);
      }
    }
#pragma unroll
    for (int j = 0; j < BC; ++j) {
      if (b0 + j < batch) {
#pragma unroll
        for (int f = 0; f < F; ++f) {
          const float t = wave_sum(acc[j][f]);
          if (lane == 0 && o0 + f < n) y[(size_t)(b0 + j) * ldy + o0 + f] = t + (bias ? bias[o0 + f] : 0.f);
        }
      }
    }
  }
}

template <bool WBF16, bool GROUPED>
__global__ __launch_bounds__(256) void skinny_mfma_kernel(const float* __restrict__ x, int ldx, int batch, int k,
                                                           const void* __restrict__ wv, const float* __restrict__ bias, int n, int act_in,
                                                           float* __restrict__ y, int ldy, const MvdSegTable seg, int xseg) {
  typedef __attribute__((ext_vector_type(16))) float f32x16;
  __shared__ f32x16 red[3][64];
  constexpr int KS = WBF16 ? 16 : 8;
  constexpr int KL = KS / 2;
  const int lane = threadIdx.x & 63, wave = threadIdx.x >> 6;
  const int li = lane & 31, h = lane >> 5;
  const int o0 = blockIdx.x * 32;
  if constexpr (GROUPED) {
    int g = 0;
    while (g + 1 < seg.n && o0 >= seg.end[g]) ++g;
    x += (size_t)g * xseg;
  }
  const int o = o0 + li < n ? o0 + li : n - 1;
  for (int b0 = 0; b0 < batch; b0 += 32) {
    const int jr = b0 + li < batch ? b0 + li : batch - 1;
    const float* xr = x + (size_t)jr * ldx;
    f32x16 acc;
#pragma unroll
    for (int r = 0; r < 16; ++r) acc[r] = 0.f;
#pragma unroll 4
    for (int kc = wave * KS; kc < k; kc += 4 * KS) {
      const bool live = kc + h * KL < k;
      const int kk = live ? kc + h * KL : kc;
      float wf[KL], xf[KL];
      if constexpr (WBF16) {
// ... 15 lines not shown
      for (int e = 0; e < KL; ++e) acc = __builtin_amdgcn_mfma_f32_32x32x2f32(wf[e], xf[e], acc, 0, 0, 0);
    }
    if (wave) red[wave - 1][lane] = acc;
    __syncthreads();
    if (wave == 0) {
#pragma unroll
      for (int w = 0; w < 3; ++w) {
        const f32x16 t = red[w][lane];
#pragma unroll
        for (int r = 0; r < 16; ++r) acc[r] += t[r];
      }
      if (b0 + li < batch) {
        float* yr = y + (size_t)(b0 + li) * ldy;
#pragma unroll
        for (int r = 0; r < 16; ++r) {
          const int oo = o0 + 8 * (r >> 2) + 4 * h + (r & 3);
          if (oo < n) yr[oo] = acc[r] + (bias ? bias[oo] : 0.f);
        }
      }
    }
    __syncthreads();
  }
}

__global__ void timestep_embedding_kernel(const float* __restrict__ t, int dim, float* __restrict__ y) {
  const int b = blockIdx.x;
  const int half = dim >> 1;
  for (int i = threadIdx.x; i < half; i += blockDim.x) {
    const float f = expf(-9.210340371976184f * (float)i / (float)half);
    const float ang = t[b] * f;
    y[(size_t)b * dim + i] = cosf(ang);
    y[(size_t)b * dim + half + i] = sinf(ang);
  }
}

__global__ void camera_features_kernel(const float* __restrict__ src, const float* __restrict__ tgt, int cam_rows,
                                       int nfreq, float log_max_freq, float* __restrict__ rflat,
                                       float* __restrict__ enc) {
  const int b = blockIdx.x;
  __shared__ float R[9], T[3];
  const float* s = src + (size_t)b * cam_rows * 4;
  const float* g = tgt + (size_t)b * cam_rows * 4;
  if (threadIdx.x < 9) {
    const int i = threadIdx.x / 3, j = threadIdx.x % 3;
    float a = 0.f;
    for (int kk = 0; kk < 3; ++kk) a += g[i * 4 + kk] * s[j * 4 + kk];
    R[threadIdx.x] = a;
    rflat[(size_t)b * 9 + threadIdx.x] = a;
  }
  __syncthreads();
  if (threadIdx.x < 3) {
    const int i = threadIdx.x;
    float a = g[i * 4 + 3];
    for (int kk = 0; kk < 3; ++kk) a -= R[i * 3 + kk] * s[kk * 4 + 3];
    T[i] = a;
  }
  __syncthreads();
  for (int e = threadIdx.x; e < 3 * nfreq; e += blockDim.x) {
    const int ax = e / nfreq, i = e % nfreq;
    const float f = expf(log_max_freq * (float)i / (float)(nfreq - 1));
    const float ang = T[ax] * f;
    enc[(size_t)b * 6 * nfreq + ax * 2 * nfreq + i] = sinf(ang);
    enc[(size_t)b * 6 * nfreq + ax * 2 * nfreq + nfreq + i] = cosf(ang);
  }
}

__global__ void film_params_kernel(const float* __restrict__ raw, int batch, int dim, float strength, float* __restrict__ scale,
                                   float* __restrict__ shift, int total) {
  const int i = blockIdx.x * blockDim.x + threadIdx.x;
  if (i >= total) return;
  const int b = (i / dim) % batch, ch = i % dim;
  const float s = raw[(size_t)b * 2 * dim + ch], t = raw[(size_t)b * 2 * dim + dim + ch];
  scale[i] = 2.0f * strength / (1.0f + expf(-s));
  shift[i] = t * strength;
}

template <int CIN>
__global__ void im2col_in_kernel(const float* __restrict__ x, int h, int w, const float* __restrict__ scale,
                                 const float* __restrict__ shift, int ld_ss, bf16_t* __restrict__ y, long total) {
  const long i = (long)blockIdx.x * blockDim.x + threadIdx.x;
  if (i >= total) return;
  const int hw = h * w;
  const int p = i % hw;
  const int b = i / hw;
  const int oy = p / w, ox = p % w;
  float v[64];
#pragma unroll
  for (int k = 0; k < 64; ++k) v[k] = 0.f;
#pragma unroll
  for (int tap = 0; tap < 9; ++tap) {
    const int iy = oy + tap / 3 - 1, ix = ox + tap % 3 - 1;
    const bool ok = (unsigned)iy < (unsigned)h && (unsigned)ix < (unsigned)w;
#pragma unroll
    for (int ch = 0; ch < CIN; ++ch) {
      if (ok) {
        float t = x[((size_t)b * CIN + ch) * hw + iy * w + ix];
        if (scale) t = t * scale[(size_t)b * ld_ss + ch] + shift[(size_t)b * ld_ss + ch];
        v[tap * CIN + ch] = t;
      }
    }
  }
  u32x4* out = reinterpret_cast<u32x4*>(y + i * 64);
#pragma unroll
  for (int q = 0; q < 8; ++q)
    out[q] = u32x4{pack2bf(v[8 * q], v[8 * q + 1]), pack2bf(v[8 * q + 2], v[8 * q + 3]), pack2bf(v[8 * q + 4], v[8 * q + 5]),
                   pack2bf(v[8 * q + 6], v[8 * q + 7])};
}

__global__ void film_nchw_f32_kernel(const float* __restrict__ x, int c, int hw, const float* __restrict__ scale,
                                     const float* __restrict__ shift, float* __restrict__ y, long total) {
  const long i = (long)blockIdx.x * blockDim.x + threadIdx.x;
  if (i >= total) return;
  const long bc = i / hw;
  y[i] = fmaf(x[i], scale[bc], shift[bc]);
}

inline int nblk(long n, int t) { return (int)((n + t - 1) / t); }

}

int mvd_launch_nchw_to_nhwc(const float* x, int batch, int c, int hw, const float* scale, const float* shift, int ld_ss,
                            bf16_t* y, hipStream_t s) {
  if (!x || !y || batch <= 0 || c <= 0 || hw <= 0 || ((scale == nullptr) != (shift == nullptr))) { mvd_set_error("nchw_to_nhwc: bad arguments"); return -1; }
  const long total = (long)batch * c * hw;
  hipLaunchKernelGGL(nchw_to_nhwc_kernel, dim3(nblk(total, 256)), dim3(256), 0, s, x, c, hw, scale, shift, ld_ss, y, total);
  return launch_check("nchw_to_nhwc");
}

int mvd_launch_nhwc_to_nchw_f32(const bf16_t* x, int batch, int hw, int c, float* y, hipStream_t s) {
  if (!x || !y || batch <= 0 || c <= 0 || hw <= 0) { mvd_set_error("nhwc_to_nchw: bad arguments"); return -1; }
  const long total = (long)batch * c * hw;
  hipLaunchKernelGGL(nhwc_to_nchw_f32_kernel, dim3(nblk(total, 256)), dim3(256), 0, s, x, hw, c, y, total);
  return launch_check("nhwc_to_nchw");
}

int mvd_launch_film(const bf16_t* x, int batch, int hw, int c, const float* scale, const float* shift, int ld_ss,
                    bf16_t* y, hipStream_t s) {
  if (!x || !y || !scale || !shift || batch <= 0 || hw <= 0 || c <= 0 || (c % 8)) { mvd_set_error("film: bad arguments"); return -1; }
  const long nvec = (long)batch * hw * (c / 8);
  int grid = nblk(nvec, 256);
  if (grid > 4096) grid = 4096;
  hipLaunchKernelGGL(film_kernel, dim3(grid), dim3(256), 0, s, x, hw, c, scale, shift, ld_ss, y, nvec);
  return launch_check("film");
}

int mvd_launch_conv_in(const bf16_t* x, int batch, int h, int w, int cin, const float* wt, const float* bias, int cout,
                       bf16_t* y, hipStream_t s) {
  if (!x || !y || !wt || !bias || batch <= 0 || h <= 0 || w <= 0 || cin <= 0 || cin > 16 || (cout % 8)) { mvd_set_error("conv_in: bad arguments"); return -1; }
  const long total = (long)batch * h * w * (cout / 8);
  hipLaunchKernelGGL(conv_in_kernel, dim3(nblk(total, 256)), dim3(256), 0, s, x, h, w, cin, wt, bias, cout, y, total);
  return launch_check("conv_in");
}

#ifdef MVD_PROBE
#include <stdio.h>
#include <unistd.h>
#include "probe/conv_out4.inc"
__global__ void word_sum_kernel(const unsigned* __restrict__ p, long n, unsigned long long* out) {
  unsigned long long s = 0;
  for (long i = (long)blockIdx.x * blockDim.x + threadIdx.x; i < n; i += (long)gridDim.x * blockDim.x) s += (unsigned long long)p[i] * (unsigned long long)((i & 1023) + 1);
  atomicAdd(out, s);
}
__global__ void conv_out_cmp_kernel(const float* __restrict__ a, const float* __restrict__ b, const float* __restrict__ r, long n,
                                    float tol, unsigned long long* cnt) {
  for (long i = (long)blockIdx.x * blockDim.x + threadIdx.x; i < n; i += (long)gridDim.x * blockDim.x) {
    const float va = a[i], vb = b[i], vr = r[i];
    if (__float_as_uint(va) != __float_as_uint(vb)) { __hip_atomic_fetch_add(cnt, 1ull, __ATOMIC_RELAXED, __HIP_MEMORY_SCOPE_SYSTEM); __hip_atomic_store(cnt + 3, (unsigned long long)i, __ATOMIC_RELAXED, __HIP_MEMORY_SCOPE_SYSTEM); }
    if (!(fabsf(va - vr) <= tol)) __hip_atomic_fetch_add(cnt + 1, 1ull, __ATOMIC_RELAXED, __HIP_MEMORY_SCOPE_SYSTEM);
    if (!(fabsf(vb - vr) <= tol)) __hip_atomic_fetch_add(cnt + 2, 1ull, __ATOMIC_RELAXED, __HIP_MEMORY_SCOPE_SYSTEM);
  }
}
#endif

int mvd_launch_conv_out(const bf16_t* x, int batch, int h, int w, int c, const bf16_t* wt, const float* bias, int cout,
                        float* y, hipStream_t s) {
  if (!x || !y || !wt || !bias || batch <= 0 || h <= 0 || w <= 0 || (c % 8) || cout <= 0 || cout > 8) { mvd_set_error("conv_out: bad arguments"); return -1; }
#ifdef MVD_PROBE
  if (MVD_ENV_INT("MVD_CONV_OUT4", 0)) {
    const long quads = (long)batch * h * ((w + 3) / 4);
    hipLaunchKernelGGL(conv_out4_kernel, dim3(nblk(quads, 4)), dim3(256), 0, s, x, batch, h, w, c, wt, bias, cout, y);
    if (MVD_ENV_INT("MVD_CONV_OUT_HASH", 0)) {
      static unsigned long long* dsum = nullptr; static float* y1 = nullptr; static size_t y1n = 0;
      const size_t on = (size_t)batch * cout * h * w;
      if (!dsum) (void)hipMalloc(&dsum, 3 * sizeof(unsigned long long));
      if (y1n < on) { if (y1) (void)hipFree(y1); (void)hipMalloc(&y1, on * sizeof(float)); y1n = on; }
      (void)hipMemsetAsync(dsum, 0, 3 * sizeof(unsigned long long), s);
      const long pix1 = (long)batch * h * w;
      hipLaunchKernelGGL(conv_out_kernel, dim3(nblk(pix1, 4)), dim3(256), 0, s, x, batch, h, w, c, wt, bias, cout, y1);
      hipLaunchKernelGGL(word_sum_kernel, dim3(1024), dim3(256), 0, s, reinterpret_cast<const unsigned*>(x), (long)((size_t)batch * h * w * c / 2), dsum);
      hipLaunchKernelGGL(word_sum_kernel, dim3(1024), dim3(256), 0, s, reinterpret_cast<const unsigned*>(y), (long)on, dsum + 1);
      hipLaunchKernelGGL(word_sum_kernel, dim3(1024), dim3(256), 0, s, reinterpret_cast<const unsigned*>(y1), (long)on, dsum + 2);
      unsigned long long hs[3] = {0, 0, 0};
      (void)hipMemcpyAsync(hs, dsum, sizeof(hs), hipMemcpyDeviceToHost, s);
      (void)hipStreamSynchronize(s);
      fprintf(stderr, "conv_out hash pid %d: input %016llx  out(4-pixel) %016llx  out(1-pixel, same input) %016llx\n", (int)getpid(), hs[0], hs[1], hs[2]);
    }
    if (MVD_ENV_INT("MVD_CONV_OUT_CMP", 0)) {
      static unsigned long long* cnt = nullptr; static float* yb = nullptr; static float* yr = nullptr; static size_t yn = 0;
      static unsigned long long seen[3] = {0, 0, 0}; static int calls = 0;
      const size_t on = (size_t)batch * cout * h * w;
      if (!cnt) { (void)hipHostMalloc(&cnt, 4 * sizeof(unsigned long long), hipHostMallocMapped); cnt[0] = cnt[1] = cnt[2] = cnt[3] = 0; }
      if (yn < on) { if (yb) { (void)hipFree(yb); (void)hipFree(yr); } (void)hipMalloc(&yb, on * sizeof(float)); (void)hipMalloc(&yr, on * sizeof(float)); yn = on; }
      hipLaunchKernelGGL(conv_out4_kernel, dim3(nblk(quads, 4)), dim3(256), 0, s, x, batch, h, w, c, wt, bias, cout, yb);
      hipLaunchKernelGGL(conv_out_kernel, dim3(nblk((long)batch * h * w, 4)), dim3(256), 0, s, x, batch, h, w, c, wt, bias, cout, yr);
      hipLaunchKernelGGL(conv_out_cmp_kernel, dim3(256), dim3(256), 0, s, y, yb, yr, (long)on, 1e-3f, cnt);
      ++calls;
      volatile unsigned long long* vc = cnt;
      const unsigned long long c0 = vc[0], c1 = vc[1], c2 = vc[2];
      if (c0 != seen[0] || c1 != seen[1] || c2 != seen[2] || calls == 2 || calls == 20) {
        seen[0] = c0; seen[1] = c1; seen[2] = c2;
        fprintf(stderr, "conv_out cmp pid %d after ~%d calls: first!=second %llu  |first-ref|>1e-3 %llu  |second-ref|>1e-3 %llu  last idx %llu (x mod 4 = %llu)\n",
                (int)getpid(), calls - 1, c0, c1, c2, (unsigned long long)vc[3], (unsigned long long)vc[3] % 4);
      }
    }
    return launch_check("conv_out4");
  }
#endif
  const long pix = (long)batch * h * w;
  hipLaunchKernelGGL(conv_out_kernel, dim3(nblk(pix, 4)), dim3(256), 0, s, x, batch, h, w, c, wt, bias, cout, y);
  return launch_check("conv_out");
}

int mvd_launch_f32_to_bf16(const float* x, int64_t n, bf16_t* y, hipStream_t s) {
  if (!x || !y || n <= 0) { mvd_set_error("f32_to_bf16: bad arguments"); return -1; }
  int grid = nblk(n, 256);
  if (grid > 4096) grid = 4096;
  hipLaunchKernelGGL(f32_to_bf16_kernel, dim3(grid), dim3(256), 0, s, x, (long)n, y);
  return launch_check("f32_to_bf16");
}

int mvd_launch_skinny_linear(const float* x, int ldx, int batch, int k, const void* w, int wbf16, const float* bias, int n,
                             int act_in, float* y, int ldy, hipStream_t s) {
  if (!x || !w || !y || batch <= 0 || batch > 4096 || k <= 0 || n <= 0 || ldx < k || ldy < n) { mvd_set_error("skinny_linear: bad arguments"); return -1; }
  const int kv = wbf16 ? 8 : 4;
  const bool vec = (k % kv) == 0 && (ldx % 4) == 0 && (((uintptr_t)x | (uintptr_t)w) & 15) == 0;
  static const int use_vec = MVD_ENV_INT("MVD_SKINNY_VEC", 1);
  if (vec && batch >= 8 && !(mvd_debug_flags() & MVD_DBG_SKINNY_VECTOR)) {
    const MvdSegTable none{};
    if (wbf16) hipLaunchKernelGGL((skinny_mfma_kernel<true, false>), dim3(nblk(n, 32)), dim3(256), 0, s, x, ldx, batch, k, w, bias, n, act_in, y, ldy, none, 0);
    else hipLaunchKernelGGL((skinny_mfma_kernel<false, false>), dim3(nblk(n, 32)), dim3(256), 0, s, x, ldx, batch, k, w, bias, n, act_in, y, ldy, none, 0);
    return launch_check("skinny_mfma");
  }
  if (vec && use_vec) {
    constexpr int F = 2;
    const dim3 g(nblk(n, 4 * F));
    if (wbf16) hipLaunchKernelGGL((skinny_linear_vec_kernel<true, F>), g, dim3(256), 0, s, x, ldx, batch, k, w, bias, n, act_in, y, ldy);
    else hipLaunchKernelGGL((skinny_linear_vec_kernel<false, F>), g, dim3(256), 0, s, x, ldx, batch, k, w, bias, n, act_in, y, ldy);
    return launch_check("skinny_linear");
  }
  if (wbf16) hipLaunchKernelGGL(skinny_linear_kernel<true>, dim3(nblk(n, 4)), dim3(256), 0, s, x, ldx, batch, k, w, bias, n, act_in, y, ldy);
  else hipLaunchKernelGGL(skinny_linear_kernel<false>, dim3(nblk(n, 4)), dim3(256), 0, s, x, ldx, batch, k, w, bias, n, act_in, y, ldy);
  return launch_check("skinny_linear");
}

int mvd_launch_skinny_linear_grouped(const float* x, int ldx, int xseg, int batch, int k, const float* w, const float* bias, int n,
                                     const MvdSegTable& seg, float* y, int ldy, hipStream_t s) {
  if (!x || !w || !y || batch <= 0 || batch > 4096 || k <= 0 || (k % 4) || (ldx % 4) || n <= 0 || ldy < n || seg.n < 1 || seg.n > 16 ||
      seg.end[seg.n - 1] != n || (((uintptr_t)x | (uintptr_t)w) & 15) || (xseg % 4)) { mvd_set_error("skinny_linear_grouped: bad arguments"); return -1; }
  for (int g = 0; g < seg.n; ++g) if (seg.end[g] % 2) { mvd_set_error("skinny_linear_grouped: segment ends must be even"); return -1; }
  bool tiles_ok = batch >= 8 && !(mvd_debug_flags() & MVD_DBG_SKINNY_VECTOR);
  for (int g = 0; g + 1 < seg.n; ++g) tiles_ok = tiles_ok && seg.end[g] % 32 == 0;
  if (tiles_ok) {
    hipLaunchKernelGGL((skinny_mfma_kernel<false, true>), dim3(nblk(n, 32)), dim3(256), 0, s, x, ldx, batch, k, (const void*)w, bias, n, 0, y, ldy, seg, xseg);
    return launch_check("skinny_mfma_grouped");
  }
  hipLaunchKernelGGL((skinny_linear_vec_kernel<false, 2, true>), dim3(nblk(n, 8)), dim3(256), 0, s, x, ldx, batch, k, (const void*)w, bias, n, 0, y, ldy, seg, xseg);
  return launch_check("skinny_linear_grouped");
}

__global__ void film_params_grouped_kernel(const float* __restrict__ raw, int batch, int ldraw, const MvdSegTable seg, float strength,
                                           float* __restrict__ out, int out_rows, int total) {
  const int i = blockIdx.x * blockDim.x + threadIdx.x;
  if (i >= total) return;
  const int half = seg.end[seg.n - 1] / 2;
  const int r = i / half, cc = i - r * half;
  int g = 0, c0 = 0;
  while (g + 1 < seg.n && cc >= seg.end[g] / 2) ++g;
  c0 = g ? seg.end[g - 1] / 2 : 0;
  const int dim = seg.end[g] / 2 - c0, ch = cc - c0;
  const int b = r % batch;
  const float* rw = raw + (size_t)b * ldraw + 2 * c0;
  const float sv = rw[ch], tv = rw[dim + ch];
  float* o = out + (size_t)out_rows * 2 * c0;
  o[(size_t)r * dim + ch] = 2.0f * strength / (1.0f + expf(-sv));
  o[(size_t)out_rows * dim + (size_t)r * dim + ch] = tv * strength;
}

int mvd_launch_film_params_grouped(const float* raw, int batch, const MvdSegTable& seg, float strength, float* out, int out_rows,
                                   hipStream_t s) {
  if (!raw || !out || batch <= 0 || out_rows < batch || seg.n < 1 || seg.n > 16) { mvd_set_error("film_params_grouped: bad arguments"); return -1; }
  const int total = out_rows * (seg.end[seg.n - 1] / 2);
  hipLaunchKernelGGL(film_params_grouped_kernel, dim3(nblk(total, 256)), dim3(256), 0, s, raw, batch, seg.end[seg.n - 1], seg, strength, out, out_rows, total);
  return launch_check("film_params_grouped");
}

int mvd_launch_timestep_embedding(const float* t, int batch, int dim, float* y, hipStream_t s) {
  if (!t || !y || batch <= 0 || dim <= 0 || (dim & 1)) { mvd_set_error("timestep_embedding: bad arguments"); return -1; }
  hipLaunchKernelGGL(timestep_embedding_kernel, dim3(batch), dim3(128), 0, s, t, dim, y);
  return launch_check("timestep_embedding");
}

int mvd_launch_camera_features(const float* src, const float* tgt, int batch, int cam_rows, int nfreq, float max_freq,
                               float* rflat, float* enc, hipStream_t s) {
  if (!src || !tgt || !rflat || !enc || batch <= 0 || (cam_rows != 3 && cam_rows != 4) || nfreq < 2) { mvd_set_error("camera_features: bad arguments"); return -1; }
  hipLaunchKernelGGL(camera_features_kernel, dim3(batch), dim3(256), 0, s, src, tgt, cam_rows, nfreq, logf(max_freq), rflat, enc);
  return launch_check("camera_features");
}

int mvd_launch_film_params(const float* raw, int batch, int dim, float strength, float* scale, float* shift, int out_rows,
                           hipStream_t s) {
  if (!raw || !scale || !shift || batch <= 0 || dim <= 0 || out_rows < batch) { mvd_set_error("film_params: bad arguments"); return -1; }
  const int total = out_rows * dim;
  hipLaunchKernelGGL(film_params_kernel, dim3(nblk(total, 256)), dim3(256), 0, s, raw, batch, dim, strength, scale, shift, total);
  return launch_check("film_params");
}

int mvd_launch_film_nchw_f32(const float* x, int batch, int c, int hw, const float* scale, const float* shift, float* y,
                             hipStream_t s) {
  if (!x || !y || !scale || !shift || batch <= 0 || c <= 0 || hw <= 0) { mvd_set_error("film_nchw: bad arguments"); return -1; }
  const long total = (long)batch * c * hw;
  hipLaunchKernelGGL(film_nchw_f32_kernel, dim3(nblk(total, 256)), dim3(256), 0, s, x, c, hw, scale, shift, y, total);
  return launch_check("film_nchw");
}

int mvd_launch_im2col_in(const float* x, int batch, int c, int h, int w, const float* scale, const float* shift, int ld_ss,
                         bf16_t* y, hipStream_t s) {
  if (!x || !y || batch <= 0 || c <= 0 || c > 7 || h <= 0 || w <= 0 || ((scale == nullptr) != (shift == nullptr))) { mvd_set_error("im2col_in: bad arguments (c=%d must be <= 7)", c); return -1; }
  const long total = (long)batch * h * w;
  const dim3 g(nblk(total, 128)), t(128);
  switch (c) {
    case 1: hipLaunchKernelGGL(im2col_in_kernel<1>, g, t, 0, s, x, h, w, scale, shift, ld_ss, y, total); break;
    case 2: hipLaunchKernelGGL(im2col_in_kernel<2>, g, t, 0, s, x, h, w, scale, shift, ld_ss, y, total); break;
    case 3: hipLaunchKernelGGL(im2col_in_kernel<3>, g, t, 0, s, x, h, w, scale, shift, ld_ss, y, total); break;
    case 4: hipLaunchKernelGGL(im2col_in_kernel<4>, g, t, 0, s, x, h, w, scale, shift, ld_ss, y, total); break;
    case 5: hipLaunchKernelGGL(im2col_in_kernel<5>, g, t, 0, s, x, h, w, scale, shift, ld_ss, y, total); break;
    case 6: hipLaunchKernelGGL(im2col_in_kernel<6>, g, t, 0, s, x, h, w, scale, shift, ld_ss, y, total); break;
    default: hipLaunchKernelGGL(im2col_in_kernel<7>, g, t, 0, s, x, h, w, scale, shift, ld_ss, y, total); break;
  }
  return launch_check("im2col_in");
}
```

### mvd_amd/csrc/norm.hip

```cpp
#include <stdlib.h>
#include "kernels.h"
#include "bufaddr.h"

namespace {

MVD_DEVINL void unpack8(const u32x4 v, float* f) {
  f[0] = bflo(v[0]); f[1] = bfhi(v[0]); f[2] = bflo(v[1]); f[3] = bfhi(v[1]);
  f[4] = bflo(v[2]); f[5] = bfhi(v[2]); f[6] = bflo(v[3]); f[7] = bfhi(v[3]);
}
MVD_DEVINL u32x4 pack8(const float* f) {
  return u32x4{pack2bf(f[0], f[1]), pack2bf(f[2], f[3]), pack2bf(f[4], f[5]), pack2bf(f[6], f[7])};
}

__global__ void gn_stats_kernel(const bf16_t* __restrict__ x0, const bf16_t* __restrict__ x1, int c0, int c1, int hw,
                                int groups, int rows_per_chunk, int R, float* __restrict__ ws) {
  extern __shared__ __attribute__((aligned(16))) float sh[];
  const int C = c0 + c1, vec = C >> 3;
  const int b = blockIdx.y, chunk = blockIdx.x, nchunk = gridDim.x;
  const int v = threadIdx.x % vec, r = threadIdx.x / vec;
  const int row0 = chunk * rows_per_chunk;
  const int row1 = min(hw, row0 + rows_per_chunk);
  const int ch = v * 8;
  const bool first = ch < c0;
  const bf16_t* src = first ? x0 + (size_t)b * hw * c0 + ch : x1 + (size_t)b * hw * c1 + (ch - c0);
// ... 267 lines not shown
    if (v < vec) {
#pragma unroll
      for (int j = 0; j < 8; ++j) { const float d = f[i][j] - mean; q = fmaf(d, d, q); }
    }
  }
  const float rstd = rsqrtf(wave_sum(q) / (float)c + eps);
#pragma unroll
  for (int i = 0; i < MAXV; ++i) {
    const int v = lane + i * 64;
    if (v < vec) {
      float o[8];
      const f32x4 g0 = *reinterpret_cast<const f32x4*>(gamma + v * 8), g1 = *reinterpret_cast<const f32x4*>(gamma + v * 8 + 4);
      const f32x4 b0 = *reinterpret_cast<const f32x4*>(beta + v * 8), b1 = *reinterpret_cast<const f32x4*>(beta + v * 8 + 4);
#pragma unroll
      for (int j = 0; j < 4; ++j) {
        o[j] = (f[i][j] - mean) * rstd * g0[j] + b0[j];
        o[j + 4] = (f[i][j + 4] - mean) * rstd * g1[j] + b1[j];
      }
      *reinterpret_cast<u32x4*>(y + (size_t)row * c + v * 8) = pack8(o);
    }
  }
}

__global__ __launch_bounds__(256) void refnorm_kernel(const bf16_t* __restrict__ x, int batch, int hw, int c,
                                                      bf16_t* __restrict__ y) {
  __shared__ float red[8];
  const int p = blockIdx.x;
  const int vec = c >> 3;
  const int total = batch * vec;
  const int lane = threadIdx.x & 63, wave = threadIdx.x >> 6;
  auto block_sum = [&](float v) -> float {
    v = wave_sum(v);
    __syncthreads();
    if (lane == 0) red[wave] = v;
    __syncthreads();
    return red[0] + red[1] + red[2] + red[3];
  };
  float s = 0.f;
  for (int e = threadIdx.x; e < total; e += 256) {
    const int b = e / vec, v = e % vec;
    float f[8];
    unpack8(*reinterpret_cast<const u32x4*>(x + ((size_t)b * hw + p) * c + v * 8), f);
#pragma unroll
    for (int j = 0; j < 8; ++j) s += f[j];
  }
  const float n = (float)batch * (float)c;
  const float mean = block_sum(s) / n;
  float q = 0.f;
  for (int e = threadIdx.x; e < total; e += 256) {
    const int b = e / vec, v = e % vec;
    float f[8];
    unpack8(*reinterpret_cast<const u32x4*>(x + ((size_t)b * hw + p) * c + v * 8), f);
#pragma unroll
    for (int j = 0; j < 8; ++j) { const float d = f[j] - mean; q = fmaf(d, d, q); }
  }
  const float var = block_sum(q) / (n - 1.0f);
  const float k = 0.5f / fmaxf(sqrtf(var), 1e-6f);
  for (int e = threadIdx.x; e < total; e += 256) {
    const int b = e / vec, v = e % vec;
    float f[8];
    const size_t off = ((size_t)b * hw + p) * c + v * 8;
    unpack8(*reinterpret_cast<const u32x4*>(x + off), f);
#pragma unroll
    for (int j = 0; j < 8; ++j) f[j] = (f[j] - mean) * k;
    *reinterpret_cast<u32x4*>(y + off) = pack8(f);
  }
}

__global__ __launch_bounds__(256) void refnorm_grouped_kernel(const bf16_t* __restrict__ x, int group, int hw, int c,
                                                              bf16_t* __restrict__ y) {
  __shared__ float red[8];
  const int p = blockIdx.x;
  const size_t base = (size_t)blockIdx.y * group * hw * c;
  x += base; y += base;
  const int vec = c >> 3;
  const int total = group * vec;
  const int lane = threadIdx.x & 63, wave = threadIdx.x >> 6;
  auto block_sum = [&](float v) -> float {
    v = wave_sum(v);
    __syncthreads();
    if (lane == 0) red[wave] = v;
    __syncthreads();
    return red[0] + red[1] + red[2] + red[3];
  };
  float s = 0.f;
  for (int e = threadIdx.x; e < total; e += 256) {
    const int b = e / vec, v = e % vec;
    float f[8];
    unpack8(*reinterpret_cast<const u32x4*>(x + ((size_t)b * hw + p) * c + v * 8), f);
#pragma unroll
    for (int j = 0; j < 8; ++j) s += f[j];
  }
  const float n = (float)group * (float)c;
  const float mean = block_sum(s) / n;
  float q = 0.f;
  for (int e = threadIdx.x; e < total; e += 256) {
    const int b = e / vec, v = e % vec;
    float f[8];
    unpack8(*reinterpret_cast<const u32x4*>(x + ((size_t)b * hw + p) * c + v * 8), f);
#pragma unroll
    for (int j = 0; j < 8; ++j) { const float d = f[j] - mean; q = fmaf(d, d, q); }
  }
  const float var = block_sum(q) / (n - 1.0f);
  const float k = 0.5f / fmaxf(sqrtf(var), 1e-6f);
  for (int e = threadIdx.x; e < total; e += 256) {
    const int b = e / vec, v = e % vec;
    float f[8];
    const size_t off = ((size_t)b * hw + p) * c + v * 8;
    unpack8(*reinterpret_cast<const u32x4*>(x + off), f);
#pragma unroll
    for (int j = 0; j < 8; ++j) f[j] = (f[j] - mean) * k;
    *reinterpret_cast<u32x4*>(y + off) = pack8(f);
  }
}

__global__ __launch_bounds__(256) void refstats_kernel(const bf16_t* __restrict__ x, int batch, int hw, int c, float* __restrict__ stats) {
  __shared__ float red[8];
  const int p = blockIdx.x;
  const int vec = c >> 3;
  const int total = batch * vec;
  const int lane = threadIdx.x & 63, wave = threadIdx.x >> 6;
  auto block_sum = [&](float v) -> float {
    v = wave_sum(v);
    __syncthreads();
    if (lane == 0) red[wave] = v;
    __syncthreads();
    return red[0] + red[1] + red[2] + red[3];
  };
  float s = 0.f;
  for (int e = threadIdx.x; e < total; e += 256) {
    const int b = e / vec, v = e % vec;
    float f[8];
    unpack8(*reinterpret_cast<const u32x4*>(x + ((size_t)b * hw + p) * c + v * 8), f);
#pragma unroll
    for (int j = 0; j < 8; ++j) s += f[j];
  }
  const float mean = block_sum(s) / ((float)batch * (float)c);
  float q = 0.f;
  for (int e = threadIdx.x; e < total; e += 256) {
    const int b = e / vec, v = e % vec;
    float f[8];
    unpack8(*reinterpret_cast<const u32x4*>(x + ((size_t)b * hw + p) * c + v * 8), f);
#pragma unroll
    for (int j = 0; j < 8; ++j) { const float d = f[j] - mean; q = fmaf(d, d, q); }
  }
  const float m2 = block_sum(q);
  if (threadIdx.x == 0) { stats[2 * p] = mean; stats[2 * p + 1] = m2; }
}

__global__ __launch_bounds__(256) void refapply_kernel(const bf16_t* __restrict__ x, int batch, int hw, int c,
                                                       const float* __restrict__ mean_k, bf16_t* __restrict__ y) {
  const int vec = c >> 3;
  const long total = (long)batch * hw * vec;
  for (long e = (long)blockIdx.x * 256 + threadIdx.x; e < total; e += (long)gridDim.x * 256) {
    const int p = (int)((e / vec) % hw);
    const float mean = mean_k[2 * p], k = mean_k[2 * p + 1];
    float f[8];
    unpack8(*reinterpret_cast<const u32x4*>(x + e * 8), f);
#pragma unroll
    for (int j = 0; j < 8; ++j) f[j] = (f[j] - mean) * k;
    *reinterpret_cast<u32x4*>(y + e * 8) = pack8(f);
  }
}

__global__ __launch_bounds__(256) void ln_f32_kernel(const float* __restrict__ x, int c, float eps,
                                                      const float* __restrict__ gamma, const float* __restrict__ beta,
                                                      int silu, float* __restrict__ y, int nseg) {
  __shared__ float red[8];
  const int row = blockIdx.x;
  gamma += (size_t)(row % nseg) * c; beta += (size_t)(row % nseg) * c;
  const int lane = threadIdx.x & 63, wave = threadIdx.x >> 6;
  auto block_sum = [&](float v) -> float {
    v = wave_sum(v);
    __syncthreads();
    if (lane == 0) red[wave] = v;
    __syncthreads();
    return red[0] + red[1] + red[2] + red[3];
  };
  const float* xr = x + (size_t)row * c;
  float s = 0.f;
  for (int i = threadIdx.x; i < c; i += 256) s += xr[i];
  const float mean = block_sum(s) / (float)c;
  float q = 0.f;
  for (int i = threadIdx.x; i < c; i += 256) { const float d = xr[i] - mean; q = fmaf(d, d, q); }
  const float rstd = rsqrtf(block_sum(q) / (float)c + eps);
  for (int i = threadIdx.x; i < c; i += 256) {
    float t = (xr[i] - mean) * rstd * gamma[i] + beta[i];
    y[(size_t)row * c + i] = silu ? silu_f(t) : t;
  }
}

}

static thread_local int g_last_gn[6] = {0, 0, 0, 0, 0, 0};

static int check_launch(const char* what) {
  hipError_t e = hipGetLastError();
  if (e != hipSuccess) { mvd_set_error("%s launch: %s", what, hipGetErrorString(e)); return -3; }
  return 0;
}

static bool launch_gn_slice(const bf16_t* x0, const bf16_t* x1, int c0, int c1, int batch, int hw, int groups, float eps,
                            const float* gamma, const float* beta, int silu, bf16_t* y, hipStream_t s) {
  static const int enable = MVD_ENV_INT("MVD_GN_SLICE", 1);
  const int C = c0 + c1, cg = C / groups;
  if (!enable || cg < 8 || (cg & 1)) return false;
  int gpw = 1;
  while (gpw <= groups && ((gpw * cg) % 8 || groups % gpw)) gpw <<= 1;
  if (gpw > groups) return false;
  const int cs = gpw * cg, nvec = cs / 8, nslice = groups / gpw;
  int threads = 1024, nv = 0;
  for (int th : {256, 512, 1024}) {
    const int npl = th / nvec;
    if (npl < 1) continue;
    threads = th; nv = (hw + npl - 1) / npl;
    if (nv <= 4) break;
  }
  if (nv < 1 || nv > 21) return false;
  const long slice_bytes = (long)hw * cs * 2, nwg = (long)batch * nslice;
  const long min_wg = (mvd_debug_flags() & MVD_DBG_GN_ONE_PASS) ? 8 : 128;
  if (slice_bytes > 96 * 1024 && nwg < min_wg) return false;
  const dim3 grid((unsigned)nwg), blk((unsigned)threads);
  g_last_gn[0] = 1; g_last_gn[2] = threads; g_last_gn[3] = gpw; g_last_gn[4] = threads / nvec; g_last_gn[5] = 0;
#define GN_SLICE(NVT) do { g_last_gn[1] = NVT; \
    hipLaunchKernelGGL(gn_slice_kernel<NVT>, grid, blk, 0, s, x0, x1, c0, c1, batch, hw, groups, gpw, eps, gamma, beta, silu, y); } while (0)
  if (nv <= 2) GN_SLICE(2); else if (nv <= 4) GN_SLICE(4); else if (nv <= 8) GN_SLICE(8); else if (nv <= 16) GN_SLICE(16); else GN_SLICE(21);
#undef GN_SLICE
  return true;
}

int mvd_launch_groupnorm(const bf16_t* x0, const bf16_t* x1, int c0, int c1, int batch, int hw, int groups, float eps,
                         const float* gamma, const float* beta, int silu, bf16_t* y, float* ws, hipStream_t s) {
  const int C = c0 + c1;
  if (!x0 || (c1 && !x1) || !y || !ws || !gamma || !beta || batch <= 0 || hw <= 0 || groups <= 0 || groups > 32 ||
      (C % groups) || (c0 % 8) || (c1 % 8) || C > 8192) {
    mvd_set_error("groupnorm: bad arguments (c0=%d c1=%d batch=%d hw=%d groups=%d)", c0, c1, batch, hw, groups);
    return -1;
  }
  if (launch_gn_slice(x0, x1, c0, c1, batch, hw, groups, eps, gamma, beta, silu, y, s)) return check_launch("gn_slice");
  const int vec = C / 8;
  if (vec > 1024) { mvd_set_error("groupnorm: C=%d too wide", C); return -1; }
  const int R = vec >= 256 ? 1 : 256 / vec;
  const int threads = ((vec * R + 63) / 64) * 64;
  static const int rows_target = MVD_ENV_INT("MVD_GN_ROWS", 128);
  int nchunk = hw / rows_target;
#ifndef MVD_GN_MINBLOCKS
#define MVD_GN_MINBLOCKS 64
#endif
  if ((long)nchunk * batch < MVD_GN_MINBLOCKS) nchunk = (MVD_GN_MINBLOCKS + batch - 1) / batch;
  if (nchunk > hw / 8) nchunk = hw / 8;
  nchunk = nchunk < 1 ? 1 : (nchunk > MVD_GN_MAXCHUNK ? MVD_GN_MAXCHUNK : nchunk);
  const int rpc = (hw + nchunk - 1) / nchunk;
  nchunk = (hw + rpc - 1) / rpc;
  const size_t sh1 = (size_t)R * C * 2 * sizeof(float);
  hipLaunchKernelGGL(gn_stats_kernel, dim3(nchunk, batch), dim3(threads), sh1, s, x0, x1, c0, c1, hw, groups, rpc, R, ws);
  if (int r = check_launch("gn_stats")) return r;
  static const long per_blk_env = MVD_ENV_INT("MVD_GN_APPLY_ELEMS", 65536);
  long per_blk = per_blk_env;
  const long total_el = (long)batch * hw * C;
  if (total_el / per_blk < 1024) per_blk = total_el / 1024 < 2048 ? 2048 : total_el / 1024;
  int rows_per_blk = (int)((per_blk + C - 1) / C);
  if (rows_per_blk < 1) rows_per_blk = 1;
  if (rows_per_blk > hw) rows_per_blk = hw;
  const int nblk = (hw + rows_per_blk - 1) / rows_per_blk;
  const size_t sh2 = (size_t)(2 * groups + 2 * C) * sizeof(float);
  g_last_gn[0] = 2; g_last_gn[1] = R; g_last_gn[2] = threads; g_last_gn[3] = nchunk; g_last_gn[4] = rpc; g_last_gn[5] = rows_per_blk;
  hipLaunchKernelGGL(gn_apply_kernel, dim3(nblk, batch), dim3(256), sh2, s, x0, x1, c0, c1, hw, groups, nchunk, rpc, eps, gamma,
                     beta, silu, ws, rows_per_blk, y);
  return check_launch("gn_apply");
}

extern "C" int mvd_debug_last_groupnorm_plan(int* out) {
  if (!out) { mvd_set_error("last_groupnorm_plan: null argument"); return -1; }
  for (int i = 0; i < 6; ++i) out[i] = g_last_gn[i];
  return 0;
}

int mvd_launch_layernorm(const bf16_t* x, int rows, int c, float eps, const float* gamma, const float* beta, bf16_t* y,
                         hipStream_t s) {
  if (!x || !y || !gamma || !beta || rows <= 0 || c <= 0 || (c % 8) || c > 64 * 8 * 4) {
    mvd_set_error("layernorm: bad arguments rows=%d c=%d", rows, c);
    return -1;
  }
  const int grid = (rows + 3) / 4;
  if (c <= 512) hipLaunchKernelGGL(ln_kernel<1>, dim3(grid), dim3(256), 0, s, x, rows, c, eps, gamma, beta, y);
  else if (c <= 1024) hipLaunchKernelGGL(ln_kernel<2>, dim3(grid), dim3(256), 0, s, x, rows, c, eps, gamma, beta, y);
  else hipLaunchKernelGGL(ln_kernel<4>, dim3(grid), dim3(256), 0, s, x, rows, c, eps, gamma, beta, y);
  return check_launch("layernorm");
}

int mvd_launch_refstats(const bf16_t* x, int batch, int hw, int c, float* stats, hipStream_t s) {
  if (!x || !stats || batch <= 0 || hw <= 0 || c <= 0 || (c % 8)) { mvd_set_error("refstats: bad arguments"); return -1; }
  hipLaunchKernelGGL(refstats_kernel, dim3(hw), dim3(256), 0, s, x, batch, hw, c, stats);
  return check_launch("refstats");
}
int mvd_launch_refapply(const bf16_t* x, int batch, int hw, int c, const float* mean_k, bf16_t* y, hipStream_t s) {
  if (!x || !y || !mean_k || batch <= 0 || hw <= 0 || c <= 0 || (c % 8)) { mvd_set_error("refapply: bad arguments"); return -1; }
  const long total = (long)batch * hw * (c >> 3);
  long grid = (total + 255) / 256; if (grid > 4096) grid = 4096;
  hipLaunchKernelGGL(refapply_kernel, dim3((unsigned)grid), dim3(256), 0, s, x, batch, hw, c, mean_k, y);
  return check_launch("refapply");
}
int mvd_launch_refnorm(const bf16_t* x, int batch, int hw, int c, bf16_t* y, hipStream_t s) {
  if (!x || !y || batch <= 0 || hw <= 0 || c <= 0 || (c % 8)) { mvd_set_error("refnorm: bad arguments"); return -1; }
  hipLaunchKernelGGL(refnorm_kernel, dim3(hw), dim3(256), 0, s, x, batch, hw, c, y);
  return check_launch("refnorm");
}

int mvd_launch_refnorm_grouped(const bf16_t* x, int batch, int group, int hw, int c, bf16_t* y, hipStream_t s) {
  if (!x || !y || batch <= 0 || hw <= 0 || c <= 0 || (c % 8)) { mvd_set_error("refnorm_grouped: bad arguments"); return -1; }
  if (group <= 0 || batch % group) { mvd_set_error("refnorm_grouped: group %d does not divide the batch %d", group, batch); return -1; }
  if (batch / group > 65535) { mvd_set_error("refnorm_grouped: %d groups exceed the grid", batch / group); return -1; }
  hipLaunchKernelGGL(refnorm_grouped_kernel, dim3(hw, batch / group), dim3(256), 0, s, x, group, hw, c, y);
  return check_launch("refnorm_grouped");
}

int mvd_launch_layernorm_f32(const float* x, int rows, int c, float eps, const float* gamma, const float* beta, int silu,
                             float* y, hipStream_t s, int nseg) {
  if (!x || !y || !gamma || !beta || rows <= 0 || c <= 0 || nseg < 1) { mvd_set_error("layernorm_f32: bad arguments"); return -1; }
  hipLaunchKernelGGL(ln_f32_kernel, dim3(rows), dim3(256), 0, s, x, c, eps, gamma, beta, silu, y, nseg);
  return check_launch("layernorm_f32");
}
```

### mvd_amd/csrc/probe/conv_out4.inc

```
__global__ __launch_bounds__(256) void conv_out4_kernel(const bf16_t* __restrict__ x, int batch, int h, int w, int c,
                                                        const bf16_t* __restrict__ wt, const float* __restrict__ bias,
                                                        int cout, float* __restrict__ y) {
  constexpr int PX = 4;
  const int lane = threadIdx.x & 63;
  const int wq = (w + PX - 1) / PX;
  const long quad = (long)blockIdx.x * 4 + (threadIdx.x >> 6);
  const int hw = h * w;
  if (quad >= (long)batch * h * wq) return;
  const int b = (int)(quad / ((long)h * wq));
  const int r = (int)(quad - (long)b * h * wq);
  const int oy = r / wq, ox0 = (r - oy * wq) * PX;
  const int vec = c >> 3;
  float acc[PX][8];
#pragma unroll
  for (int p = 0; p < PX; ++p)
#pragma unroll
    for (int j = 0; j < 8; ++j) acc[p][j] = 0.f;
  for (int q = lane; q < 3 * vec; q += 64) {
    const int dy = q / vec, v = q - dy * vec;
    const int iy = oy + dy - 1;
    if ((unsigned)iy >= (unsigned)h) continue;
    u32x4 xv[PX + 2];
#pragma unroll
    for (int k = 0; k < PX + 2; ++k) {
      const int ix = ox0 + k - 1;
      xv[k] = u32x4{0u, 0u, 0u, 0u};
      if ((unsigned)ix < (unsigned)w) xv[k] = *reinterpret_cast<const u32x4*>(x + ((size_t)b * hw + iy * w + ix) * c + v * 8);
    }
#pragma unroll
    for (int co = 0; co < 8; ++co) {
      if (co < cout) {
#pragma unroll
        for (int dx = 0; dx < 3; ++dx) {
          const u32x4 wv = *reinterpret_cast<const u32x4*>(wt + ((size_t)co * 9 + dy * 3 + dx) * c + v * 8);
#pragma unroll
          for (int p = 0; p < PX; ++p) {
            float a = acc[p][co];
#pragma unroll
            for (int j = 0; j < 4; ++j) {
              a = fmaf(bflo(xv[p + dx][j]), bflo(wv[j]), a);
              a = fmaf(bfhi(xv[p + dx][j]), bfhi(wv[j]), a);
            }
            acc[p][co] = a;
          }
        }
      }
    }
  }
#pragma unroll
  for (int co = 0; co < 8; ++co) {
    if (co < cout) {
#pragma unroll
      for (int p = 0; p < PX; ++p) {
        const float t = wave_sum(acc[p][co]);
        if (lane == 0 && ox0 + p < w) y[((size_t)b * cout + co) * hw + oy * w + ox0 + p] = t + bias[co];
      }
    }
  }
}
```

### mvd_amd/ops.py

```python
from __future__ import annotations

import ctypes as C
from typing import Optional

import torch

from . import _lib as L


def _p(t: Optional[torch.Tensor]):
    if t is None:
        return None
    assert t.is_cuda and t.is_contiguous(), "ops expect contiguous CUDA tensors"
    return C.c_void_p(t.data_ptr())


_s = L.stream


def _bf16(*ts):
    for t in ts:
        if t is not None:
            assert t.dtype == torch.bfloat16, "expected bf16"

# ... 243 lines not shown
    return out


def inception_score_chunks(logits, perm, splits):
    assert logits.dtype == torch.float32 and logits.dim() == 2 and perm.dtype == torch.int32 and perm.shape == (logits.shape[0],)
    n, classes = logits.shape
    need = L.lib().mvd_op_inception_score_workspace_bytes(n, classes, int(splits))
    if need < 0:
        raise L.MvdError(f"mvd_op_inception_score_workspace_bytes: {L.last_error()}")
    ws = torch.empty(need, dtype=torch.uint8, device=logits.device)
    out = torch.empty(min(int(splits), n), dtype=torch.float64, device=logits.device)
    chunks = C.c_int(0)
    L.call("mvd_op_inception_score", _p(logits), n, classes, _p(perm), int(splits), _p(ws), need, _p(out), C.byref(chunks), _s())
    return out[:chunks.value]


def knn_radii(f, k, force_parts=0, want_list=False, ws=None):
    assert f.dtype == torch.float32 and f.dim() == 2
    n, d = f.shape
    need = L.lib().mvd_op_knn_radii_workspace_bytes(n, int(k), int(force_parts))
    if need < 0:
        raise L.MvdError(f"mvd_op_knn_radii_workspace_bytes: {L.last_error()}")
    if ws is None:
        ws = torch.empty(need, dtype=torch.uint8, device=f.device)
    radii = torch.empty(n, dtype=torch.float64, device=f.device)
    knn = torch.empty(n, int(k) + 1, dtype=torch.float64, device=f.device) if want_list else None
    L.call("mvd_op_knn_radii", _p(f), n, d, int(k), int(force_parts), _p(radii), _p(knn), _p(ws), need, _s())
    return (radii, knn) if want_list else radii


def manifold_counts(q, r, radii_sq, closed, want_query=True, want_ref=True):
    assert q.dtype == torch.float32 and r.dtype == torch.float32 and q.dim() == 2 and r.dim() == 2 and q.shape[1] == r.shape[1]
    assert radii_sq.dtype == torch.float64 and radii_sq.shape == (r.shape[0],)
    hq = torch.empty(q.shape[0], dtype=torch.int32, device=q.device) if want_query else None
    hr = torch.empty(r.shape[0], dtype=torch.int32, device=q.device) if want_ref else None
    L.call("mvd_op_manifold_counts", _p(q), q.shape[0], _p(r), r.shape[0], q.shape[1], _p(radii_sq), int(bool(closed)), _p(hq), _p(hr), _s())
    return hq, hr


def up4_launches() -> int:
    return int(L.lib().mvd_debug_up4_launches())


def attention(q, k, v, heads, scale=0.125):
    _bf16(q, k, v)
    B, nq, _ = q.shape
    nk = k.shape[1]
    assert q.stride(2) == 1 and k.stride(2) == 1 and v.stride(2) == 1
    assert q.stride(0) == nq * q.stride(1) and k.stride(0) == nk * k.stride(1) and v.stride(0) == nk * v.stride(1)
    out = torch.empty(B, nq, heads * 64, device=q.device, dtype=torch.bfloat16)
    L.call("mvd_op_attention", C.c_void_p(q.data_ptr()), C.c_void_p(k.data_ptr()), C.c_void_p(v.data_ptr()), _p(out),
           B, heads, nq, nk, q.stride(1), k.stride(1), v.stride(1), heads * 64, float(scale), _s())
    return out


def attention_grouped(q, k, v, heads, kv_group, scale=0.125):
    _bf16(q, k, v)
    B, nq, _ = q.shape
    nk = k.shape[1]
    assert kv_group >= 1 and B % kv_group == 0 and k.shape[0] == B // kv_group and v.shape[0] == B // kv_group, (B, kv_group, k.shape, v.shape)
    assert q.stride(2) == 1 and k.stride(2) == 1 and v.stride(2) == 1
    assert q.stride(0) == nq * q.stride(1) and k.stride(0) == nk * k.stride(1) and v.stride(0) == nk * v.stride(1)
    out = torch.empty(B, nq, heads * 64, device=q.device, dtype=torch.bfloat16)
    L.call("mvd_op_attention_grouped", C.c_void_p(q.data_ptr()), C.c_void_p(k.data_ptr()), C.c_void_p(v.data_ptr()), _p(out),
           B, heads, nq, nk, q.stride(1), k.stride(1), v.stride(1), heads * 64, float(scale), int(kv_group), _s())
    return out


def attention_objects(q, k, v, heads, kv_group, kv_objects, scale=0.125):
    _bf16(q, k, v)
    B, nq, _ = q.shape
    nk = k.shape[1]
    kvg = max(int(kv_group), 1)
    assert kv_objects >= 0 and B % (kvg * max(int(kv_objects), 1)) == 0 and k.shape[0] == B // kvg and v.shape[0] == B // kvg, (B, kv_group, kv_objects, k.shape, v.shape)
    assert q.stride(2) == 1 and k.stride(2) == 1 and v.stride(2) == 1
    assert q.stride(0) == nq * q.stride(1) and k.stride(0) == nk * k.stride(1) and v.stride(0) == nk * v.stride(1)
    out = torch.empty(B, nq, heads * 64, device=q.device, dtype=torch.bfloat16)
    L.call("mvd_op_attention_objects", C.c_void_p(q.data_ptr()), C.c_void_p(k.data_ptr()), C.c_void_p(v.data_ptr()), _p(out),
           B, heads, nq, nk, q.stride(1), k.stride(1), v.stride(1), heads * 64, float(scale), int(kv_group), int(kv_objects), _s())
    return out


def attention_mapped(q, k, v, heads, kv_index, scale=0.125):
    _bf16(q, k, v)
    B, nq, _ = q.shape
    nk = k.shape[1]
    idx = [int(i) for i in (kv_index.tolist() if isinstance(kv_index, torch.Tensor) else kv_index)]
    if isinstance(kv_index, torch.Tensor):
        assert not kv_index.is_cuda and not kv_index.is_floating_point(), "kv_index: a CPU int tensor"
    assert len(idx) == B and k.shape[0] == v.shape[0], (B, len(idx), k.shape, v.shape)
    assert q.stride(2) == 1 and k.stride(2) == 1 and v.stride(2) == 1
    assert q.stride(0) == nq * q.stride(1) and k.stride(0) == nk * k.stride(1) and v.stride(0) == nk * v.stride(1)
    out = torch.empty(B, nq, heads * 64, device=q.device, dtype=torch.bfloat16)
    L.call("mvd_op_attention_mapped", C.c_void_p(q.data_ptr()), C.c_void_p(k.data_ptr()), C.c_void_p(v.data_ptr()), _p(out),
           B, heads, nq, nk, q.stride(1), k.stride(1), v.stride(1), heads * 64, float(scale), (C.c_int * B)(*idx), int(k.shape[0]), _s())
    return out


def attention_causal(q, k, v, heads, scale=0.125):
    _bf16(q, k, v)
    B, n, _ = q.shape
    assert k.shape[1] == n and v.shape[1] == n
    assert q.stride(2) == 1 and k.stride(2) == 1 and v.stride(2) == 1
    assert q.stride(0) == n * q.stride(1) and k.stride(0) == n * k.stride(1) and v.stride(0) == n * v.stride(1)
    out = torch.empty(B, n, heads * 64, device=q.device, dtype=torch.bfloat16)
    L.call("mvd_op_attention_causal", C.c_void_p(q.data_ptr()), C.c_void_p(k.data_ptr()), C.c_void_p(v.data_ptr()), _p(out),
           B, heads, n, q.stride(1), k.stride(1), v.stride(1), heads * 64, float(scale), _s())
    return out


def attention_split(q, k, v, heads, nsplit):
    _bf16(q, k, v)
    B, nq, _ = q.shape
    nk = k.shape[1]
    out = torch.empty(B, nq, heads * 64, device=q.device, dtype=torch.bfloat16)
    ws = torch.empty(int(L.lib().mvd_op_attention_split_ws_bytes(B, heads, nq, nsplit)), device=q.device, dtype=torch.uint8)
    L.call("mvd_op_attention_split", C.c_void_p(q.data_ptr()), C.c_void_p(k.data_ptr()), C.c_void_p(v.data_ptr()), _p(out),
           B, heads, nq, nk, q.stride(1), k.stride(1), v.stride(1), heads * 64, nsplit, _p(ws), _s())
    return out


def groupnorm(x, gamma, beta, groups=32, eps=1e-5, silu=False, x2=None):
    _bf16(x, x2)
    B, hw, c0 = x.shape
    c1 = x2.shape[2] if x2 is not None else 0
    y = torch.empty(B, hw, c0 + c1, device=x.device, dtype=torch.bfloat16)
    ws = torch.empty(B * 256 * groups * 2, device=x.device, dtype=torch.float32)
    L.call("mvd_op_groupnorm", _p(x), _p(x2), c0, c1, B, hw, groups, float(eps), _p(gamma), _p(beta), int(silu), _p(y),
           _p(ws), _s())
    return y


def layernorm(x, gamma, beta, eps=1e-5):
    _bf16(x)
    rows, c = x.shape
    y = torch.empty_like(x)
    L.call("mvd_op_layernorm", _p(x), rows, c, float(eps), _p(gamma), _p(beta), _p(y), _s())
    return y


def refnorm(x):
    _bf16(x)
    B, hw, c = x.shape
    y = torch.empty_like(x)
    L.call("mvd_op_refnorm", _p(x), B, hw, c, _p(y), _s())
    return y


def refnorm_grouped(x, group):
    _bf16(x)
    B, hw, c = x.shape
    y = torch.empty_like(x)
    L.call("mvd_op_refnorm_grouped", _p(x), B, int(group), hw, c, _p(y), _s())
    return y


def film(x, scale, shift):
    _bf16(x)
    B, hw, c = x.shape
    y = torch.empty_like(x)
    L.call("mvd_op_film", _p(x), B, hw, c, _p(scale), _p(shift), _p(y), _s())
    return y


def conv_in(x, w, bias):
    B, H, W, cin = x.shape
    cout = w.shape[0]
    y = torch.empty(B, H, W, cout, device=x.device, dtype=torch.bfloat16)
    L.call("mvd_op_conv_in", _p(x), B, H, W, cin, _p(w), _p(bias), cout, _p(y), _s())
    return y


def conv_out(x, w, bias):
    B, H, W, c = x.shape
    cout = w.shape[0]
    y = torch.empty(B, cout, H, W, device=x.device, dtype=torch.float32)
    L.call("mvd_op_conv_out", _p(x), B, H, W, c, _p(w), _p(bias), cout, _p(y), _s())
    return y


def softmax_rows(s):
    assert s.dtype == torch.float32 and s.dim() == 2
    out = torch.empty(s.shape, device=s.device, dtype=torch.bfloat16)
    L.call("mvd_op_softmax_rows", _p(s), s.shape[0], s.shape[1], _p(out), _s())
    return out


def ddpm_step(model_out, sample, noise, c0, c1, c2, c3, sigma):
    assert model_out.dtype == torch.float32 and sample.dtype == torch.float32
    out = torch.empty_like(sample)
    L.call("mvd_op_ddpm_step", _p(model_out), _p(sample), _p(noise), float(c0), float(c1), float(c2), float(c3),
           float(sigma), _p(out), sample.numel(), _s())
    return out


def cfg_combine(uncond_cond, guidance_scale):
    assert uncond_cond.dtype == torch.float32 and uncond_cond.shape[0] % 2 == 0
    out = torch.empty((uncond_cond.shape[0] // 2,) + tuple(uncond_cond.shape[1:]), device=uncond_cond.device,
                      dtype=torch.float32)
    L.call("mvd_op_cfg_combine", _p(uncond_cond), float(guidance_scale), _p(out), out.numel(), _s())
    return out


def sampler_step(model_out, sample, a0, a1, p, q, r=0.0, sigma=0.0, x0_prev=None, noise=None, guidance_scale=None,
                 out=None, x0_out=None):
    guided = guidance_scale is not None
    assert model_out.dtype == torch.float32 and sample.dtype == torch.float32
    assert model_out.numel() == sample.numel() * (2 if guided else 1), (tuple(model_out.shape), tuple(sample.shape))
    for t in (x0_prev, noise, out, x0_out):
        assert t is None or (t.dtype == torch.float32 and t.numel() == sample.numel())
    if out is None:
        out = torch.empty_like(sample)
    L.call("mvd_op_sampler_step", _p(model_out), int(guided), float(guidance_scale) if guided else 0.0, _p(sample), _p(x0_prev),
           _p(noise), float(a0), float(a1), float(p), float(q), float(r), float(sigma), _p(out), _p(x0_out), sample.numel(), _s())
    return out


def _rescale_rows(uncond_cond):
    if uncond_cond.dim() < 2 or uncond_cond.shape[0] % 2:
        raise L.MvdError(f"guidance rescale: expected [uncond | cond] of shape (2 * rows, ...), got {tuple(uncond_cond.shape)}")
    if not (uncond_cond.is_cuda and uncond_cond.dtype == torch.float32 and uncond_cond.is_contiguous()):
        raise L.MvdError(f"guidance rescale: expected a contiguous fp32 CUDA tensor, got {uncond_cond.dtype} on {uncond_cond.device}")
    rows = uncond_cond.shape[0] // 2
    return rows, uncond_cond.numel() // (2 * rows)


def cfg_rescale(uncond_cond, guidance_scale, guidance_rescale, out=None):
    rows, n_row = _rescale_rows(uncond_cond)
    if out is None:
        out = torch.empty((rows,) + tuple(uncond_cond.shape[1:]), device=uncond_cond.device, dtype=torch.float32)
    assert out.dtype == torch.float32 and out.numel() == rows * n_row and out.is_contiguous()
    L.call("mvd_op_cfg_rescale", _p(uncond_cond), float(guidance_scale), float(guidance_rescale), _p(out), rows, n_row, _s())
    return out


def sampler_step_rescaled(model_out, sample, guidance_scale, guidance_rescale, a0, a1, p, q, r=0.0, sigma=0.0, x0_prev=None,
                          noise=None, out=None, x0_out=None):
    rows, n_row = _rescale_rows(model_out)
    assert sample.dtype == torch.float32 and sample.numel() == rows * n_row, (tuple(model_out.shape), tuple(sample.shape))
    for t in (x0_prev, noise, out, x0_out):
        assert t is None or (t.dtype == torch.float32 and t.numel() == sample.numel())
    if out is None:
        out = torch.empty_like(sample)
    L.call("mvd_op_sampler_step_rescaled", _p(model_out), float(guidance_scale), float(guidance_rescale), _p(sample), _p(x0_prev),
           _p(noise), float(a0), float(a1), float(p), float(q), float(r), float(sigma), _p(out), _p(x0_out), rows, n_row, _s())
    return out


def cfg_rescale_plan(n_row):
    out = (C.c_int * 4)()
    L.call("mvd_debug_cfg_rescale_plan", int(n_row), out)
    per_pass = out[0] * out[1]
    return dict(threads=out[0], vec=out[1], wave=out[2], keep=out[3], passes=-(-int(n_row) // per_pass))


def cfg_rescale_partition(n_row):
    plan = cfg_rescale_plan(n_row)
    n_row, vec, wchunk = int(n_row), plan["vec"], plan["wave"] * plan["vec"]
    offs = set(range(wchunk, n_row, wchunk))
    offs.update(range(vec, min(wchunk, n_row), vec))
    last = (n_row - 1) // wchunk * wchunk
    offs.update(range(last + vec, n_row, vec))
    return sorted(offs)


APG_SPACES = ("output", "x0")


def _apg_momentum(momentum, momentum_buffer, rows, n_row):
    if float(momentum) == 0.0 or momentum_buffer is None:
        return None
    if not (momentum_buffer.is_cuda and momentum_buffer.dtype == torch.float32 and momentum_buffer.is_contiguous()
            and momentum_buffer.numel() == rows * n_row):
        raise L.MvdError(f"apg: momentum_buffer must be a contiguous fp32 CUDA tensor of {rows} x {n_row} floats, got "
                         f"{tuple(momentum_buffer.shape)} {momentum_buffer.dtype} on {momentum_buffer.device}")
    return momentum_buffer


def apg(uncond_cond, guidance_scale, eta=0.0, norm_threshold=0.0, momentum=0.0, guidance_rescale=0.0, momentum_buffer=None,
        out=None):
    rows, n_row = _rescale_rows(uncond_cond)
    if out is None:
        out = torch.empty((rows,) + tuple(uncond_cond.shape[1:]), device=uncond_cond.device, dtype=torch.float32)
    assert out.dtype == torch.float32 and out.numel() == rows * n_row and out.is_contiguous()
    L.call("mvd_op_apg", _p(uncond_cond), float(guidance_scale), float(eta), float(norm_threshold), float(momentum),
           float(guidance_rescale), _p(_apg_momentum(momentum, momentum_buffer, rows, n_row)), _p(out), rows, n_row, _s())
    return out


def sampler_step_apg(model_out, sample, guidance_scale, a0, a1, p, q, r=0.0, sigma=0.0, eta=0.0, norm_threshold=0.0, momentum=0.0,
                     guidance_rescale=0.0, space="output", momentum_buffer=None, x0_prev=None, noise=None, out=None, x0_out=None):
    rows, n_row = _rescale_rows(model_out)
    if space not in APG_SPACES:
        raise L.MvdError(f"sampler_step_apg: space={space!r}: expected one of {APG_SPACES}")
    assert sample.dtype == torch.float32 and sample.numel() == rows * n_row, (tuple(model_out.shape), tuple(sample.shape))
    for t in (x0_prev, noise, out, x0_out):
        assert t is None or (t.dtype == torch.float32 and t.numel() == sample.numel())
    if out is None:
        out = torch.empty_like(sample)
    L.call("mvd_op_sampler_step_apg", _p(model_out), float(guidance_scale), float(eta), float(norm_threshold), float(momentum),
           float(guidance_rescale), APG_SPACES.index(space), _p(_apg_momentum(momentum, momentum_buffer, rows, n_row)), _p(sample),
           _p(x0_prev), _p(noise), float(a0), float(a1), float(p), float(q), float(r), float(sigma), _p(out), _p(x0_out), rows, n_row,
           _s())
    return out


# ... 73 lines not shown
def image_metrics(x, y, data_range, ssim=True, per_image=False):
    _f32_same(x, y)
    if x.dim() != 4:
        raise L.MvdError(f"image_metrics: expected (N, C, H, W), got {tuple(x.shape)}")
    n, c, h, w = x.shape
    nbytes = L.check(L.lib().mvd_op_image_metrics_ws_bytes(n, c, h, w, int(ssim)), "mvd_op_image_metrics_ws_bytes")
    ws = torch.empty(nbytes, device=x.device, dtype=torch.uint8)
    result = torch.empty(3, device=x.device, dtype=torch.float32)
    pi = torch.empty(n, 2, device=x.device, dtype=torch.float32) if per_image else None
    L.call("mvd_op_image_metrics", _p(x), _p(y), n, c, h, w, float(data_range), int(ssim), _p(result), _p(pi), _p(ws), nbytes, _s())
    return result, pi


def _rows(t):
    assert t.dtype == torch.float32 and t.is_cuda and t.dim() == 2 and (t.shape[1] == 1 or t.stride(1) == 1), "rows must be dense fp32"
    return C.c_void_p(t.data_ptr()), (t.stride(0) if t.shape[0] > 1 else max(t.stride(0), t.shape[1]))


def skinny_linear(x, w, bias=None, silu_in=False, out=None):
    assert x.dim() == 2 and w.dim() == 2 and w.shape[1] == x.shape[1]
    assert w.dtype in (torch.float32, torch.bfloat16) and w.is_contiguous()
    b, k = x.shape
    n = w.shape[0]
    y = torch.empty(b, n, device=x.device, dtype=torch.float32) if out is None else out
    assert tuple(y.shape) == (b, n)
    (xp, ldx), (yp, ldy) = _rows(x), _rows(y)
    L.call("mvd_op_skinny_linear", xp, ldx, b, k, _p(w), int(w.dtype == torch.bfloat16), _p(bias), n, int(silu_in), yp, ldy, _s())
    return y


def _seg(seg_end):
    return (C.c_int * len(seg_end))(*[int(v) for v in seg_end]), len(seg_end)


def skinny_linear_grouped(x, w, seg_end, bias=None, xseg=None):
    assert w.dtype == torch.float32 and w.dim() == 2 and w.is_contiguous() and x.dim() == 2
    n, k = w.shape
    b = x.shape[0]
    y = torch.empty(b, n, device=x.device, dtype=torch.float32)
    xp, ldx = _rows(x)
    se, ns = _seg(seg_end)
    xseg = k if xseg is None else int(xseg)
    assert xseg >= 0 and (ns - 1) * xseg + k <= x.shape[1] and (bias is None or bias.numel() == n), "a segment's input lies outside the row"
    L.call("mvd_op_skinny_linear_grouped", xp, ldx, xseg, b, k, _p(w), _p(bias), n, se, ns, _p(y), n, _s())
    return y


def timestep_embedding(t, dim):
    assert t.dtype == torch.float32 and t.dim() == 1
    y = torch.empty(t.shape[0], dim, device=t.device, dtype=torch.float32)
    L.call("mvd_op_timestep_embedding", _p(t), t.shape[0], int(dim), _p(y), _s())
    return y


def camera_features(src, tgt, nfreq, max_freq=10.0):
    assert src.dtype == torch.float32 and tgt.dtype == torch.float32 and src.shape == tgt.shape and src.dim() == 3 and src.shape[2] == 4
    b, rows = src.shape[0], src.shape[1]
    rflat = torch.empty(b, 9, device=src.device, dtype=torch.float32)
    enc = torch.empty(b, 6 * nfreq, device=src.device, dtype=torch.float32)
    L.call("mvd_op_camera_features", _p(src), _p(tgt), b, rows, int(nfreq), float(max_freq), _p(rflat), _p(enc), _s())
    return rflat, enc


def layernorm_f32(x, gamma, beta, eps=1e-5, silu=False, nseg=1):
    assert x.dtype == torch.float32 and x.dim() == 2 and gamma.numel() == nseg * x.shape[1] and beta.numel() == nseg * x.shape[1]
    y = torch.empty_like(x)
    L.call("mvd_op_layernorm_f32", _p(x), x.shape[0], x.shape[1], float(eps), _p(gamma), _p(beta), int(silu), int(nseg), _p(y), _s())
    return y


def film_params(raw, strength, out_rows=None):
    assert raw.dtype == torch.float32 and raw.dim() == 2 and raw.shape[1] % 2 == 0
    b, dim = raw.shape[0], raw.shape[1] // 2
    rows = b if out_rows is None else int(out_rows)
    scale = torch.empty(rows, dim, device=raw.device, dtype=torch.float32)
    shift = torch.empty(rows, dim, device=raw.device, dtype=torch.float32)
    L.call("mvd_op_film_params", _p(raw), b, dim, float(strength), _p(scale), _p(shift), rows, _s())
    return scale, shift


def film_params_grouped(raw, seg_end, strength, out_rows=None):
    assert raw.dtype == torch.float32 and raw.dim() == 2 and raw.shape[1] == seg_end[-1]
    b = raw.shape[0]
    rows = b if out_rows is None else int(out_rows)
    out = torch.empty(rows * seg_end[-1], device=raw.device, dtype=torch.float32)
    se, ns = _seg(seg_end)
    L.call("mvd_op_film_params_grouped", _p(raw), b, se, ns, float(strength), _p(out), rows, _s())
    return out


def im2col_in(x, scale=None, shift=None, ld_ss=0):
    assert x.dtype == torch.float32 and x.dim() == 4
    B, c, H, W = x.shape
    if scale is not None:
        need = (B - 1) * ld_ss + c
        assert scale.dtype == torch.float32 and shift.dtype == torch.float32 and scale.numel() >= need and shift.numel() >= need
    y = torch.empty(B, H, W, 64, device=x.device, dtype=torch.bfloat16)
    L.call("mvd_op_im2col_in", _p(x), B, c, H, W, _p(scale), _p(shift), int(ld_ss), _p(y), _s())
    return y


def film_nchw_f32(x, scale, shift):
    assert x.dtype == torch.float32 and x.dim() == 3 and tuple(scale.shape) == tuple(x.shape[:2]) == tuple(shift.shape)
    assert scale.dtype == torch.float32 and shift.dtype == torch.float32
    y = torch.empty_like(x)
    L.call("mvd_op_film_nchw_f32", _p(x), x.shape[0], x.shape[1], x.shape[2], _p(scale), _p(shift), _p(y), _s())
    return y


def nchw_to_nhwc(x, scale=None, shift=None):
    B, c, H, W = x.shape
    y = torch.empty(B, H, W, c, device=x.device, dtype=torch.bfloat16)
    L.call("mvd_op_nchw_to_nhwc", _p(x), B, c, H * W, _p(scale), _p(shift), _p(y), _s())
    return y


def nhwc_to_nchw(x):
    _bf16(x)
    B, H, W, c = x.shape
    y = torch.empty(B, c, H, W, device=x.device, dtype=torch.float32)
    L.call("mvd_op_nhwc_to_nchw", _p(x), B, H * W, c, _p(y), _s())
    return y


def f32_to_bf16(x):
    assert x.dtype == torch.float32
    y = torch.empty(x.shape, device=x.device, dtype=torch.bfloat16)
    L.call("mvd_op_f32_to_bf16", _p(x), x.numel(), _p(y), _s())
    return y


def last_gemm_plan():
    out = (C.c_int * 5)()
    L.call("mvd_debug_last_gemm_plan", out)
    return dict(cfg=out[0], splitk=out[1], tiles=out[2], grid=out[3], per_cu=out[4], nowait=L.lib().mvd_debug_last_gemm_nowait())


def last_attention_plan():
    out = (C.c_int * 2)()
    L.call("mvd_debug_last_attention_plan", out)
    return dict(waves=out[0], workgroups=out[1])


def last_groupnorm_plan():
    out = (C.c_int * 6)()
    L.call("mvd_debug_last_groupnorm_plan", out)
    if out[0] == 1:
        return dict(form="slice", nv=out[1], threads=out[2], gpw=out[3], npl=out[4])
    if out[0] == 2:
        return dict(form="two_kernel", R=out[1], threads=out[2], nchunk=out[3], rows_per_chunk=out[4], apply_rows=out[5])
    return dict(form="none")


def engine_splitk(m, n, k, geglu=False, conv=False):
    if conv:
        return L.lib().mvd_debug_pick_splitk_conv(m, n, k)
    return L.lib().mvd_debug_pick_splitk(m, n, k, int(geglu))


def engine_dense_route(m, n, k1, k2=0):
    out = (C.c_int * 5)()
    L.call("mvd_debug_dense_route", m, n, k1, k2, out)
    sm = bool(out[0])
    return dict(sm=sm, cfg=out[1], splitk=out[2], depth=out[3], walk_cg=out[4], force_cfg=100 + 10 * out[1] + out[3] if sm else -1)
```

Measured before the change: 543.8 forward-passes/s.

## Tile conv_out over pixel runs with LDS weights; add register-resident refnorm kernels

The output convolution kernel is rewritten so each wave computes a run of 4-8 adjacent output pixels for all output channels. Weights are staged in LDS in channel chunks, and partial sums are reduced with a butterfly shuffle fold instead of per-channel wave sums. Separately, refnorm and refstats gain a single-pass kernel that keeps each pixel's vectors in registers across a team of threads, replacing the three-pass reduction when the data fits. The refapply index math is also made incremental, and new op and debug entry points are exported. The aim is to cut redundant global weight loads and reduction overhead, at the cost of more register pressure and many template instantiations.

After: 546.8 forward-passes/s, median of 6. No clear change (+0.6%).

```diff
diff --git a/include/mvd_hip.h b/include/mvd_hip.h
--- a/include/mvd_hip.h
+++ b/include/mvd_hip.h
@@ -136,6 +136,8 @@
                      void* stream);
 int mvd_op_refnorm(const void* x, int batch, int hw, int c, void* y, void* stream);
 int mvd_op_refnorm_grouped(const void* x, int batch, int group, int hw, int c, void* y, void* stream);
+int mvd_op_refstats(const void* x, int batch, int hw, int c, float* stats, void* stream);
+int mvd_op_refapply(const void* x, int batch, int hw, int c, const float* mean_k, void* y, void* stream);
 int mvd_op_film(const void* x, int batch, int hw, int c, const float* scale, const float* shift, void* y, void* stream);
 int mvd_op_conv_in(const void* x, int batch, int h, int w, int cin, const float* wt, const float* bias, int cout, void* y,
                    void* stream);
@@ -165,6 +167,8 @@
 int mvd_debug_last_gemm_plan(int* out);
 int mvd_debug_last_attention_plan(int* out);
 int mvd_debug_last_groupnorm_plan(int* out);
+int mvd_debug_refnorm_plan(int rows, int c, int* out);
+int mvd_debug_refnorm_three_pass(const void* x, int batch, int group, int hw, int c, void* y, void* stream);
 long mvd_debug_up4_launches(void);
 int mvd_debug_last_gemm_nowait(void);
 int mvd_debug_pick_splitk(int m, int n, int k, int geglu);
diff --git a/mvd_amd/_lib.py b/mvd_amd/_lib.py
--- a/mvd_amd/_lib.py
+++ b/mvd_amd/_lib.py
@@ -148,6 +148,8 @@
     "mvd_op_layernorm": (C.c_int, [C.c_void_p, C.c_int, C.c_int, C.c_float, C.c_void_p, C.c_void_p, C.c_void_p, C.c_void_p]),
     "mvd_op_refnorm": (C.c_int, [C.c_void_p, C.c_int, C.c_int, C.c_int, C.c_void_p, C.c_void_p]),
     "mvd_op_refnorm_grouped": (C.c_int, [C.c_void_p, C.c_int, C.c_int, C.c_int, C.c_int, C.c_void_p, C.c_void_p]),
+    "mvd_op_refstats": (C.c_int, [C.c_void_p, C.c_int, C.c_int, C.c_int, C.c_void_p, C.c_void_p]),
+    "mvd_op_refapply": (C.c_int, [C.c_void_p, C.c_int, C.c_int, C.c_int, C.c_void_p, C.c_void_p, C.c_void_p]),
     "mvd_op_film": (C.c_int, [C.c_void_p, C.c_int, C.c_int, C.c_int, C.c_void_p, C.c_void_p, C.c_void_p, C.c_void_p]),
     "mvd_op_conv_in": (C.c_int, [C.c_void_p, C.c_int, C.c_int, C.c_int, C.c_int, C.c_void_p, C.c_void_p, C.c_int, C.c_void_p, C.c_void_p]),
     "mvd_op_conv_out": (C.c_int, [C.c_void_p, C.c_int, C.c_int, C.c_int, C.c_int, C.c_void_p, C.c_void_p, C.c_int, C.c_void_p, C.c_void_p]),
@@ -174,6 +176,8 @@
     "mvd_debug_last_gemm_nowait": (C.c_int, []),
     "mvd_debug_last_attention_plan": (C.c_int, [C.POINTER(C.c_int)]),
     "mvd_debug_last_groupnorm_plan": (C.c_int, [C.POINTER(C.c_int)]),
+    "mvd_debug_refnorm_plan": (C.c_int, [C.c_int, C.c_int, C.POINTER(C.c_int)]),
+    "mvd_debug_refnorm_three_pass": (C.c_int, [C.c_void_p, C.c_int, C.c_int, C.c_int, C.c_int, C.c_void_p, C.c_void_p]),
     "mvd_debug_pick_splitk": (C.c_int, [C.c_int, C.c_int, C.c_int, C.c_int]),
     "mvd_debug_pick_splitk_conv": (C.c_int, [C.c_int, C.c_int, C.c_int]),
     "mvd_debug_dense_route": (C.c_int, [C.c_int, C.c_int, C.c_int, C.c_int, C.POINTER(C.c_int)]),
diff --git a/mvd_amd/csrc/engine.hip b/mvd_amd/csrc/engine.hip
--- a/mvd_amd/csrc/engine.hip
+++ b/mvd_amd/csrc/engine.hip
@@ -1721,6 +1721,12 @@
 int mvd_op_refnorm_grouped(const void* x, int batch, int group, int hw, int c, void* y, void* stream) {
   return mvd_launch_refnorm_grouped((const bf16_t*)x, batch, group, hw, c, (bf16_t*)y, (hipStream_t)stream);
 }
+int mvd_op_refstats(const void* x, int batch, int hw, int c, float* stats, void* stream) {
+  return mvd_launch_refstats((const bf16_t*)x, batch, hw, c, stats, (hipStream_t)stream);
+}
+int mvd_op_refapply(const void* x, int batch, int hw, int c, const float* mean_k, void* y, void* stream) {
+  return mvd_launch_refapply((const bf16_t*)x, batch, hw, c, mean_k, (bf16_t*)y, (hipStream_t)stream);
+}
 int mvd_op_film(const void* x, int batch, int hw, int c, const float* scale, const float* shift, void* y, void* stream) {
   return mvd_launch_film((const bf16_t*)x, batch, hw, c, scale, shift, c, (bf16_t*)y, (hipStream_t)stream);
 }
diff --git a/mvd_amd/csrc/misc.hip b/mvd_amd/csrc/misc.hip
--- a/mvd_amd/csrc/misc.hip
+++ b/mvd_amd/csrc/misc.hip
@@ -83,43 +83,102 @@
   *reinterpret_cast<u32x4*>(y + bp * cout + g * 8) = o;
 }
 
+template <int N, int O>
+MVD_DEVINL void conv_out_fold(float* acc, int lane) {
+  if constexpr (O >= 1) {
+    if constexpr (N > 1) {
+      const bool upper = lane & O;
+#pragma unroll
+      for (int i = 0; i < N / 2; ++i) {
+        const float send = upper ? acc[i] : acc[i + N / 2];
+        const float keep = upper ? acc[i + N / 2] : acc[i];
+        acc[i] = keep + __shfl_xor(send, O, 64);
+      }
+      conv_out_fold<N / 2, O / 2>(acc, lane);
+    } else {
+      acc[0] += __shfl_xor(acc[0], O, 64);
+      conv_out_fold<1, O / 2>(acc, lane);
+    }
+  }
+}
+
+template <int COUT>
 __global__ __launch_bounds__(256) void conv_out_kernel(const bf16_t* __restrict__ x, int batch, int h, int w, int c,
                                                         const bf16_t* __restrict__ wt, const float* __restrict__ bias,
-                                                        int cout, float* __restrict__ y) {
+                                                        float* __restrict__ y, int ck, int runs_per_wave) {
+  constexpr int R = COUT <= 4 ? 8 : 4, LR = COUT <= 4 ? 3 : 2;
+  constexpr int CP = COUT <= 1 ? 1 : COUT <= 2 ? 2 : COUT <= 4 ? 4 : 8;
+  constexpr int NACC = CP * R;
+  constexpr int SH = NACC == 32 ? 1 : NACC == 16 ? 2 : 3;
+  extern __shared__ __attribute__((aligned(16))) u32x4 wsh[];
   const int lane = threadIdx.x & 63;
-  const long pix = (long)blockIdx.x * 4 + (threadIdx.x >> 6);
   const int hw = h * w;
-  if (pix >= (long)batch * hw) return;
-  const int b = pix / hw, p = pix % hw;
-  const int oy = p / w, ox = p % w;
-  const int vec = c >> 3;
-  float acc[8];
-#pragma unroll
-  for (int j = 0; j < 8; ++j) acc[j] = 0.f;
-  for (int q = lane; q < 9 * vec; q += 64) {
-    const int tap = q / vec, v = q % vec;
-    const int iy = oy + tap / 3 - 1, ix = ox + tap % 3 - 1;
-    if ((unsigned)iy >= (unsigned)h || (unsigned)ix >= (unsigned)w) continue;
-    const u32x4 xv = *reinterpret_cast<const u32x4*>(x + ((size_t)b * hw + iy * w + ix) * c + v * 8);
-#pragma unroll
-    for (int co = 0; co < 8; ++co) {
-      if (co < cout) {
-        const u32x4 wv = *reinterpret_cast<const u32x4*>(wt + ((size_t)co * 9 + tap) * c + v * 8);
-        float a = acc[co];
-#pragma unroll
-        for (int j = 0; j < 4; ++j) {
-          a = fmaf(bflo(xv[j]), bflo(wv[j]), a);
-          a = fmaf(bfhi(xv[j]), bfhi(wv[j]), a);
+  const int rw = (w + R - 1) / R;
+  const long nruns = (long)batch * h * rw;
+  const long run0 = ((long)blockIdx.x * 4 + (threadIdx.x >> 6)) * runs_per_wave;
+  const long run1 = run0 + runs_per_wave < nruns ? run0 + runs_per_wave : nruns;
+  for (int c0 = 0; c0 < c; c0 += ck) {
+    const int vck = (c - c0 < ck ? c - c0 : ck) >> 3;
+    if (c0) __syncthreads();
+    if (vck * 8 == c) {
+      for (int i = threadIdx.x; i < COUT * 9 * vck; i += 256) wsh[i] = reinterpret_cast<const u32x4*>(wt)[i];
+    } else {
+      for (int i = threadIdx.x; i < COUT * 9 * vck; i += 256) {
+        const int row = i / vck, col = i - row * vck;
+        wsh[i] = *reinterpret_cast<const u32x4*>(wt + (size_t)row * c + c0 + col * 8);
+      }
+    }
+    __syncthreads();
+    if (run0 >= run1) continue;
+    int b, oy, rx;
+    { const long row = run0 / rw; rx = (int)(run0 - row * rw); b = (int)(row / h); oy = (int)(row - (long)b * h); }
+    const int qs = 64 / vck, rs = 64 - qs * vck;
+    const int dy0 = lane / vck, v0 = lane - dy0 * vck;
+    for (long run = run0; run < run1; ++run) {
+      const int ox0 = rx * R;
+      float acc[NACC];
+#pragma unroll
+      for (int i = 0; i < NACC; ++i) acc[i] = 0.f;
+      for (int dy = dy0, v = v0; dy < 3;) {
+        const int iy = oy + dy - 1;
+        if ((unsigned)iy < (unsigned)h) {
+          const bf16_t* xr = x + ((size_t)b * hw + (size_t)iy * w) * c + c0 + v * 8;
+          u32x4 xv[R + 2];
+#pragma unroll
+          for (int k = 0; k < R + 2; ++k) {
+            const int ix = ox0 + k - 1;
+            xv[k] = u32x4{0u, 0u, 0u, 0u};
+            if ((unsigned)ix < (unsigned)w) xv[k] = *reinterpret_cast<const u32x4*>(xr + (size_t)ix * c);
+          }
+          const u32x4* wrow = wsh + (dy * 3) * vck + v;
+#pragma unroll
+          for (int co = 0; co < COUT; ++co) {
+#pragma unroll
+            for (int dx = 0; dx < 3; ++dx) {
+              const u32x4 wv = wrow[(co * 9 + dx) * vck];
+#pragma unroll
+              for (int px = 0; px < R; ++px) {
+                float a = acc[co * R + px];
+#pragma unroll
+                for (int j = 0; j < 4; ++j) {
+                  a = fmaf(bflo(xv[px + dx][j]), bflo(wv[j]), a);
+                  a = fmaf(bfhi(xv[px + dx][j]), bfhi(wv[j]), a);
+                }
+                acc[co * R + px] = a;
+              }
+            }
+          }
         }
-        acc[co] = a;
-      }
-    }
-  }
-#pragma unroll
-  for (int co = 0; co < 8; ++co) {
-    if (co < cout) {
-      const float t = wave_sum(acc[co]);
-      if (lane == 0) y[((size_t)b * cout + co) * hw + p] = t + bias[co];
+        dy += qs; v += rs;
+        if (v >= vck) { v -= vck; ++dy; }
+      }
+      conv_out_fold<NACC, 32>(acc, lane);
+      const int idx = lane >> SH, co = idx >> LR, ox = ox0 + (idx & (R - 1));
+      if ((lane & ((1 << SH) - 1)) == 0 && co < COUT && ox < w) {
+        float* yp = y + ((size_t)b * COUT + co) * hw + (size_t)oy * w + ox;
+        *yp = c0 ? *yp + acc[0] : acc[0] + bias[co];
+      }
+      if (++rx == rw) { rx = 0; if (++oy == h) { oy = 0; ++b; } }
     }
   }
 }
@@ -441,72 +500,23 @@
   return launch_check("conv_in");
 }
 
-#ifdef MVD_PROBE
-#include <stdio.h>
-#include <unistd.h>
-#include "probe/conv_out4.inc"
-__global__ void word_sum_kernel(const unsigned* __restrict__ p, long n, unsigned long long* out) {
-  unsigned long long s = 0;
-  for (long i = (long)blockIdx.x * blockDim.x + threadIdx.x; i < n; i += (long)gridDim.x * blockDim.x) s += (unsigned long long)p[i] * (unsigned long long)((i & 1023) + 1);
-  atomicAdd(out, s);
-}
-__global__ void conv_out_cmp_kernel(const float* __restrict__ a, const float* __restrict__ b, const float* __restrict__ r, long n,
-                                    float tol, unsigned long long* cnt) {
-  for (long i = (long)blockIdx.x * blockDim.x + threadIdx.x; i < n; i += (long)gridDim.x * blockDim.x) {
-    const float va = a[i], vb = b[i], vr = r[i];
-    if (__float_as_uint(va) != __float_as_uint(vb)) { __hip_atomic_fetch_add(cnt, 1ull, __ATOMIC_RELAXED, __HIP_MEMORY_SCOPE_SYSTEM); __hip_atomic_store(cnt + 3, (unsigned long long)i, __ATOMIC_RELAXED, __HIP_MEMORY_SCOPE_SYSTEM); }
-    if (!(fabsf(va - vr) <= tol)) __hip_atomic_fetch_add(cnt + 1, 1ull, __ATOMIC_RELAXED, __HIP_MEMORY_SCOPE_SYSTEM);
-    if (!(fabsf(vb - vr) <= tol)) __hip_atomic_fetch_add(cnt + 2, 1ull, __ATOMIC_RELAXED, __HIP_MEMORY_SCOPE_SYSTEM);
-  }
-}
-#endif
-
 int mvd_launch_conv_out(const bf16_t* x, int batch, int h, int w, int c, const bf16_t* wt, const float* bias, int cout,
                         float* y, hipStream_t s) {
   if (!x || !y || !wt || !bias || batch <= 0 || h <= 0 || w <= 0 || (c % 8) || cout <= 0 || cout > 8) { mvd_set_error("conv_out: bad arguments"); return -1; }
-#ifdef MVD_PROBE
-  if (MVD_ENV_INT("MVD_CONV_OUT4", 0)) {
-    const long quads = (long)batch * h * ((w + 3) / 4);
-    hipLaunchKernelGGL(conv_out4_kernel, dim3(nblk(quads, 4)), dim3(256), 0, s, x, batch, h, w, c, wt, bias, cout, y);
-    if (MVD_ENV_INT("MVD_CONV_OUT_HASH", 0)) {
-      static unsigned long long* dsum = nullptr; static float* y1 = nullptr; static size_t y1n = 0;
-      const size_t on = (size_t)batch * cout * h * w;
-      if (!dsum) (void)hipMalloc(&dsum, 3 * sizeof(unsigned long long));
-      if (y1n < on) { if (y1) (void)hipFree(y1); (void)hipMalloc(&y1, on * sizeof(float)); y1n = on; }
-      (void)hipMemsetAsync(dsum, 0, 3 * sizeof(unsigned long long), s);
-      const long pix1 = (long)batch * h * w;
-      hipLaunchKernelGGL(conv_out_kernel, dim3(nblk(pix1, 4)), dim3(256), 0, s, x, batch, h, w, c, wt, bias, cout, y1);
-      hipLaunchKernelGGL(word_sum_kernel, dim3(1024), dim3(256), 0, s, reinterpret_cast<const unsigned*>(x), (long)((size_t)batch * h * w * c / 2), dsum);
-      hipLaunchKernelGGL(word_sum_kernel, dim3(1024), dim3(256), 0, s, reinterpret_cast<const unsigned*>(y), (long)on, dsum + 1);
-      hipLaunchKernelGGL(word_sum_kernel, dim3(1024), dim3(256), 0, s, reinterpret_cast<const unsigned*>(y1), (long)on, dsum + 2);
-      unsigned long long hs[3] = {0, 0, 0};
-      (void)hipMemcpyAsync(hs, dsum, sizeof(hs), hipMemcpyDeviceToHost, s);
-      (void)hipStreamSynchronize(s);
-      fprintf(stderr, "conv_out hash pid %d: input %016llx  out(4-pixel) %016llx  out(1-pixel, same input) %016llx\n", (int)getpid(), hs[0], hs[1], hs[2]);
-    }
-    if (MVD_ENV_INT("MVD_CONV_OUT_CMP", 0)) {
-      static unsigned long long* cnt = nullptr; static float* yb = nullptr; static float* yr = nullptr; static size_t yn = 0;
-      static unsigned long long seen[3] = {0, 0, 0}; static int calls = 0;
-      const size_t on = (size_t)batch * cout * h * w;
-      if (!cnt) { (void)hipHostMalloc(&cnt, 4 * sizeof(unsigned long long), hipHostMallocMapped); cnt[0] = cnt[1] = cnt[2] = cnt[3] = 0; }
-      if (yn < on) { if (yb) { (void)hipFree(yb); (void)hipFree(yr); } (void)hipMalloc(&yb, on * sizeof(float)); (void)hipMalloc(&yr, on * sizeof(float)); yn = on; }
-      hipLaunchKernelGGL(conv_out4_kernel, dim3(nblk(quads, 4)), dim3(256), 0, s, x, batch, h, w, c, wt, bias, cout, yb);
-      hipLaunchKernelGGL(conv_out_kernel, dim3(nblk((long)batch * h * w, 4)), dim3(256), 0, s, x, batch, h, w, c, wt, bias, cout, yr);
-      hipLaunchKernelGGL(conv_out_cmp_kernel, dim3(256), dim3(256), 0, s, y, yb, yr, (long)on, 1e-3f, cnt);
-      ++calls;
-      volatile unsigned long long* vc = cnt;
-      const unsigned long long c0 = vc[0], c1 = vc[1], c2 = vc[2];
-      if (c0 != seen[0] || c1 != seen[1] || c2 != seen[2] || calls == 2 || calls == 20) {
-        seen[0] = c0; seen[1] = c1; seen[2] = c2;
-        fprintf(stderr, "conv_out cmp pid %d after ~%d calls: first!=second %llu  |first-ref|>1e-3 %llu  |second-ref|>1e-3 %llu  last idx %llu (x mod 4 = %llu)\n",
-                (int)getpid(), calls - 1, c0, c1, c2, (unsigned long long)vc[3], (unsigned long long)vc[3] % 4);
-      }
-    }
-    return launch_check("conv_out4");
-  }
-#endif
-  const long pix = (long)batch * h * w;
-  hipLaunchKernelGGL(conv_out_kernel, dim3(nblk(pix, 4)), dim3(256), 0, s, x, batch, h, w, c, wt, bias, cout, y);
+  int ck = (48 * 1024 / (cout * 18)) & ~7;
+  if (ck > c) ck = c;
+  const size_t lds = (size_t)cout * 9 * ck * sizeof(bf16_t);
+  const int R = cout <= 4 ? 8 : 4;
+  const long nruns = (long)batch * h * ((w + R - 1) / R);
+  const long per_wave = (nruns + 4 * 1024 - 1) / (4 * 1024);
+  if (per_wave > 0x7fffffff) { mvd_set_error("conv_out: image too large"); return -1; }
+  const dim3 grid((unsigned)nblk(nblk(nruns, (int)per_wave), 4));
+#define CONV_OUT(CO) hipLaunchKernelGGL(conv_out_kernel<CO>, grid, dim3(256), lds, s, x, batch, h, w, c, wt, bias, y, ck, (int)per_wave)
+  switch (cout) {
+    case 1: CONV_OUT(1); break; case 2: CONV_OUT(2); break; case 3: CONV_OUT(3); break; case 4: CONV_OUT(4); break;
+    case 5: CONV_OUT(5); break; case 6: CONV_OUT(6); break; case 7: CONV_OUT(7); break; default: CONV_OUT(8); break;
+  }
+#undef CONV_OUT
   return launch_check("conv_out");
 }
 
diff --git a/mvd_amd/csrc/norm.hip b/mvd_amd/csrc/norm.hip
--- a/mvd_amd/csrc/norm.hip
+++ b/mvd_amd/csrc/norm.hip
@@ -443,14 +443,132 @@
                                                        const float* __restrict__ mean_k, bf16_t* __restrict__ y) {
   const int vec = c >> 3;
   const long total = (long)batch * hw * vec;
-  for (long e = (long)blockIdx.x * 256 + threadIdx.x; e < total; e += (long)gridDim.x * 256) {
-    const int p = (int)((e / vec) % hw);
+  const int stride = (int)gridDim.x * 256;
+  const int sq = stride / vec, sv = stride - sq * vec, sp = sq % hw;
+  const long e0 = (long)blockIdx.x * 256 + threadIdx.x;
+  const long row0 = e0 / vec;
+  int v = (int)(e0 - row0 * vec), p = (int)(row0 % hw);
+  for (long e = e0; e < total; e += stride) {
     const float mean = mean_k[2 * p], k = mean_k[2 * p + 1];
     float f[8];
     unpack8(*reinterpret_cast<const u32x4*>(x + e * 8), f);
 #pragma unroll
     for (int j = 0; j < 8; ++j) f[j] = (f[j] - mean) * k;
     *reinterpret_cast<u32x4*>(y + e * 8) = pack8(f);
+    v += sv; p += sp;
+    if (v >= vec) { v -= vec; ++p; }
+    if (p >= hw) p -= hw;
+  }
+}
+
+constexpr int REFNORM_NV_MAX = 20;
+
+template <int T>
+MVD_DEVINL float ref_team_sum(const float* v, float* red) {
+  constexpr int P = 256 / T;
+  float w[P];
+#pragma unroll
+  for (int j = 0; j < P; ++j) w[j] = wave_sum(v[j]);
+  if constexpr (T == 64) {
+    return w[0] + w[1] + w[2] + w[3];
+  } else {
+    const int wt = (threadIdx.x >> 6) & (T / 64 - 1);
+    float* tr = red + (threadIdx.x / T) * 4;
+    if ((threadIdx.x & 63) == 0) {
+#pragma unroll
+      for (int j = 0; j < P; ++j) tr[wt + j * (T / 64)] = w[j];
+    }
+    __syncthreads();
+    return tr[0] + tr[1] + tr[2] + tr[3];
+  }
+}
+
+struct RefStep {
+  size_t off, row_stride, step;
+  int v, vec, rs, c;
+  MVD_DEVINL RefStep(int T, int tl, int hw, int c_, int p) : c(c_) {
+    vec = c >> 3;
+    const int qs = T / vec; rs = T - qs * vec;
+    const int b0 = tl / vec; v = tl - b0 * vec;
+    row_stride = (size_t)hw * c;
+    off = ((size_t)b0 * hw + p) * c + (size_t)v * 8;
+    step = (size_t)qs * row_stride + (size_t)rs * 8;
+  }
+  MVD_DEVINL void next() {
+    v += rs; off += step;
+    if (v >= vec) { v -= vec; off += row_stride - c; }
+  }
+};
+
+template <int T, int NV>
+MVD_DEVINL void ref_team_stats(const bf16_t* __restrict__ x, int rows, int hw, int c, int p, int tl, int mine, float* red,
+                               u32x4* r, float& mean, float& m2) {
+  RefStep st(T, tl, hw, c, p);
+#pragma unroll
+  for (int i = 0; i < NV; ++i) {
+    r[i] = u32x4{0u, 0u, 0u, 0u};
+    if (tl + i * T < mine) r[i] = *reinterpret_cast<const u32x4*>(x + st.off);
+    st.next();
+  }
+  constexpr int P = 256 / T;
+  float s[P];
+#pragma unroll
+  for (int j = 0; j < P; ++j) s[j] = 0.f;
+#pragma unroll
+  for (int i = 0; i < NV; ++i) {
+    if (tl + i * T < mine) {
+      float f[8];
+      unpack8(r[i], f);
+#pragma unroll
+      for (int j = 0; j < 8; ++j) s[i % P] += f[j];
+    }
+  }
+  mean = ref_team_sum<T>(s, red) / ((float)rows * (float)c);
+  float q[P];
+#pragma unroll
+  for (int j = 0; j < P; ++j) q[j] = 0.f;
+#pragma unroll
+  for (int i = 0; i < NV; ++i) {
+    if (tl + i * T < mine) {
+      float f[8];
+      unpack8(r[i], f);
+#pragma unroll
+      for (int j = 0; j < 8; ++j) { const float d = f[j] - mean; q[i % P] = fmaf(d, d, q[i % P]); }
+    }
+  }
+  m2 = ref_team_sum<T>(q, red + 8);
+}
+
+template <int T, int NV, bool STATS>
+__global__ __launch_bounds__(256) void refnorm_reg_kernel(const bf16_t* __restrict__ x, int rows, int hw, int c,
+                                                          bf16_t* __restrict__ y, float* __restrict__ stats) {
+  __shared__ float red[16];
+  const int tl = threadIdx.x & (T - 1);
+  const int p = blockIdx.x * (256 / T) + threadIdx.x / T;
+  const int mine = p < hw ? rows * (c >> 3) : 0;
+  const size_t base = (size_t)blockIdx.y * rows * hw * c;
+  x += base;
+  u32x4 r[NV];
+  float mean, m2;
+  ref_team_stats<T, NV>(x, rows, hw, c, p, tl, mine, red, r, mean, m2);
+  if constexpr (STATS) {
+    if (tl == 0 && mine) { stats[2 * p] = mean; stats[2 * p + 1] = m2; }
+  } else {
+    y += base;
+    const float var = m2 / ((float)rows * (float)c - 1.0f);
+    const float k = 0.5f / fmaxf(sqrtf(var), 1e-6f);
+    RefStep st(T, tl, hw, c, p);
+#pragma unroll
+    for (int i = 0; i < NV; ++i) {
+      if (tl + i * T < mine) {
+        float f[8];
+        unpack8(r[i], f);
+#pragma unroll
+        for (int j = 0; j < 8; ++j) f[j] = (f[j] - mean) * k;
+        *reinterpret_cast<u32x4*>(y + st.off) = pack8(f);
+      }
+      st.next();
+    }
   }
 }
 
@@ -580,8 +698,51 @@
   return check_launch("layernorm");
 }
 
+static void refnorm_plan(int rows, int c, int* T, int* NV) {
+  const long vecs = (long)rows * (c >> 3);
+  *T = 0; *NV = 0;
+  for (int t : {64, 128, 256}) {
+    const long nv = (vecs + t - 1) / t;
+    if (nv <= REFNORM_NV_MAX) { *T = t; *NV = nv <= 5 ? 5 : nv <= 10 ? 10 : 20; return; }
+  }
+}
+
+extern "C" int mvd_debug_refnorm_plan(int rows, int c, int* out) {
+  if (!out || rows <= 0 || c <= 0 || (c % 8)) { mvd_set_error("refnorm_plan: bad arguments"); return -1; }
+  refnorm_plan(rows, c, &out[0], &out[1]);
+  return 0;
+}
+
+extern "C" int mvd_debug_refnorm_three_pass(const void* x, int batch, int group, int hw, int c, void* y, void* stream) {
+  if (!x || !y || batch <= 0 || hw <= 0 || c <= 0 || (c % 8) || group <= 0 || batch % group || batch / group > 65535) {
+    mvd_set_error("refnorm_three_pass: bad arguments");
+    return -1;
+  }
+  if (group == batch)
+    hipLaunchKernelGGL(refnorm_kernel, dim3(hw), dim3(256), 0, (hipStream_t)stream, (const bf16_t*)x, batch, hw, c, (bf16_t*)y);
+  else
+    hipLaunchKernelGGL(refnorm_grouped_kernel, dim3(hw, batch / group), dim3(256), 0, (hipStream_t)stream, (const bf16_t*)x, group, hw, c, (bf16_t*)y);
+  return check_launch("refnorm_three_pass");
+}
+
+template <bool STATS>
+static bool launch_refnorm_reg(const bf16_t* x, int rows, int runs, int hw, int c, bf16_t* y, float* stats, hipStream_t s) {
+  int T, NV;
+  refnorm_plan(rows, c, &T, &NV);
+  if (!T) return false;
+  const int ppw = 256 / T;
+  const dim3 grid((unsigned)((hw + ppw - 1) / ppw), (unsigned)runs);
+#define REF_REG(TT, NVT) hipLaunchKernelGGL((refnorm_reg_kernel<TT, NVT, STATS>), grid, dim3(256), 0, s, x, rows, hw, c, y, stats)
+#define REF_REG_T(TT) do { if (NV == 5) REF_REG(TT, 5); else if (NV == 10) REF_REG(TT, 10); else REF_REG(TT, 20); } while (0)
+  if (T == 64) REF_REG_T(64); else if (T == 128) REF_REG_T(128); else REF_REG_T(256);
+#undef REF_REG_T
+#undef REF_REG
+  return true;
+}
+
 int mvd_launch_refstats(const bf16_t* x, int batch, int hw, int c, float* stats, hipStream_t s) {
   if (!x || !stats || batch <= 0 || hw <= 0 || c <= 0 || (c % 8)) { mvd_set_error("refstats: bad arguments"); return -1; }
+  if (launch_refnorm_reg<true>(x, batch, 1, hw, c, nullptr, stats, s)) return check_launch("refstats");
   hipLaunchKernelGGL(refstats_kernel, dim3(hw), dim3(256), 0, s, x, batch, hw, c, stats);
   return check_launch("refstats");
 }
@@ -594,6 +755,7 @@
 }
 int mvd_launch_refnorm(const bf16_t* x, int batch, int hw, int c, bf16_t* y, hipStream_t s) {
   if (!x || !y || batch <= 0 || hw <= 0 || c <= 0 || (c % 8)) { mvd_set_error("refnorm: bad arguments"); return -1; }
+  if (launch_refnorm_reg<false>(x, batch, 1, hw, c, y, nullptr, s)) return check_launch("refnorm");
   hipLaunchKernelGGL(refnorm_kernel, dim3(hw), dim3(256), 0, s, x, batch, hw, c, y);
   return check_launch("refnorm");
 }
@@ -602,6 +764,7 @@
   if (!x || !y || batch <= 0 || hw <= 0 || c <= 0 || (c % 8)) { mvd_set_error("refnorm_grouped: bad arguments"); return -1; }
   if (group <= 0 || batch % group) { mvd_set_error("refnorm_grouped: group %d does not divide the batch %d", group, batch); return -1; }
   if (batch / group > 65535) { mvd_set_error("refnorm_grouped: %d groups exceed the grid", batch / group); return -1; }
+  if (launch_refnorm_reg<false>(x, group, batch / group, hw, c, y, nullptr, s)) return check_launch("refnorm_grouped");
   hipLaunchKernelGGL(refnorm_grouped_kernel, dim3(hw, batch / group), dim3(256), 0, s, x, group, hw, c, y);
   return check_launch("refnorm_grouped");
 }
diff --git a/mvd_amd/csrc/probe/conv_out4.inc b/mvd_amd/csrc/probe/conv_out4.inc
--- a/mvd_amd/csrc/probe/conv_out4.inc
+++ /dev/null
@@ -1,60 +0,0 @@
-__global__ __launch_bounds__(256) void conv_out4_kernel(const bf16_t* __restrict__ x, int batch, int h, int w, int c,
-                                                        const bf16_t* __restrict__ wt, const float* __restrict__ bias,
-                                                        int cout, float* __restrict__ y) {
-  constexpr int PX = 4;
-  const int lane = threadIdx.x & 63;
-  const int wq = (w + PX - 1) / PX;
-  const long quad = (long)blockIdx.x * 4 + (threadIdx.x >> 6);
-  const int hw = h * w;
-  if (quad >= (long)batch * h * wq) return;
-  const int b = (int)(quad / ((long)h * wq));
-  const int r = (int)(quad - (long)b * h * wq);
-  const int oy = r / wq, ox0 = (r - oy * wq) * PX;
-  const int vec = c >> 3;
-  float acc[PX][8];
-#pragma unroll
-  for (int p = 0; p < PX; ++p)
-#pragma unroll
-    for (int j = 0; j < 8; ++j) acc[p][j] = 0.f;
-  for (int q = lane; q < 3 * vec; q += 64) {
-    const int dy = q / vec, v = q - dy * vec;
-    const int iy = oy + dy - 1;
-    if ((unsigned)iy >= (unsigned)h) continue;
-    u32x4 xv[PX + 2];
-#pragma unroll
-    for (int k = 0; k < PX + 2; ++k) {
-      const int ix = ox0 + k - 1;
-      xv[k] = u32x4{0u, 0u, 0u, 0u};
-      if ((unsigned)ix < (unsigned)w) xv[k] = *reinterpret_cast<const u32x4*>(x + ((size_t)b * hw + iy * w + ix) * c + v * 8);
-    }
-#pragma unroll
-    for (int co = 0; co < 8; ++co) {
-      if (co < cout) {
-#pragma unroll
-        for (int dx = 0; dx < 3; ++dx) {
-          const u32x4 wv = *reinterpret_cast<const u32x4*>(wt + ((size_t)co * 9 + dy * 3 + dx) * c + v * 8);
-#pragma unroll
-          for (int p = 0; p < PX; ++p) {
-            float a = acc[p][co];
-#pragma unroll
-            for (int j = 0; j < 4; ++j) {
-              a = fmaf(bflo(xv[p + dx][j]), bflo(wv[j]), a);
-              a = fmaf(bfhi(xv[p + dx][j]), bfhi(wv[j]), a);
-            }
-            acc[p][co] = a;
-          }
-        }
-      }
-    }
-  }
-#pragma unroll
-  for (int co = 0; co < 8; ++co) {
-    if (co < cout) {
-#pragma unroll
-      for (int p = 0; p < PX; ++p) {
-        const float t = wave_sum(acc[p][co]);
-        if (lane == 0 && ox0 + p < w) y[((size_t)b * cout + co) * hw + oy * w + ox0 + p] = t + bias[co];
-      }
-    }
-  }
-}
diff --git a/mvd_amd/ops.py b/mvd_amd/ops.py
--- a/mvd_amd/ops.py
+++ b/mvd_amd/ops.py
@@ -419,6 +419,23 @@
     B, hw, c = x.shape
     y = torch.empty_like(x)
     L.call("mvd_op_refnorm_grouped", _p(x), B, int(group), hw, c, _p(y), _s())
+    return y
+
+
+def refstats(x):
+    _bf16(x)
+    B, hw, c = x.shape
+    stats = torch.empty(hw, 2, device=x.device, dtype=torch.float32)
+    L.call("mvd_op_refstats", _p(x), B, hw, c, _p(stats), _s())
+    return stats
+
+
+def refapply(x, mean_k):
+    _bf16(x)
+    B, hw, c = x.shape
+    assert mean_k.dtype == torch.float32 and mean_k.shape == (hw, 2) and mean_k.is_contiguous()
+    y = torch.empty_like(x)
+    L.call("mvd_op_refapply", _p(x), B, hw, c, _p(mean_k), _p(y), _s())
     return y
 
 
@@ -798,6 +815,20 @@
     return dict(form="none")
 
 
+def refnorm_plan(rows, c):
+    out = (C.c_int * 2)()
+    L.call("mvd_debug_refnorm_plan", int(rows), int(c), out)
+    return dict(form="registers", team=out[0], nv=out[1]) if out[0] else dict(form="three_pass")
+
+
+def refnorm_three_pass(x, group=None):
+    _bf16(x)
+    B, hw, c = x.shape
+    y = torch.empty_like(x)
+    L.call("mvd_debug_refnorm_three_pass", _p(x), B, B if group is None else int(group), hw, c, _p(y), _s())
+    return y
+
+
 def engine_splitk(m, n, k, geglu=False, conv=False):
     if conv:
         return L.lib().mvd_debug_pick_splitk_conv(m, n, k)
```
